# OpenNLPLab/ACR_WSSS

Hardware: NVIDIA B200
Metric: train_imgs_per_sec (higher is better)
Workload: dtype bf16

## Files before the change

acr_wsss_b200/csrc/attn_bwd_tc.cu:

```cuda
#include "attn_tc.cuh"

using namespace acr_attn;

namespace {

constexpr int NST = 3;

struct BwdSmem {
  uint8_t k[TILE_BYTES];
  uint8_t v[TILE_BYTES];
  uint8_t q[NST][TILE_BYTES];
  uint8_t d_o[NST][TILE_BYTES];
  uint8_t p[2][TILE_BYTES];
  uint8_t ds[2][TILE_BYTES];
  uint8_t dq[2][TILE_BYTES];
  float stat[2][2][BM];
  uint64_t kv_full, kv_empty, dkv_free, qdo_full[NST], qdo_empty[NST], stat_full[2], sdp_full, sdp_free, pds_full, pds_free, dq_full, dq_free;
  uint32_t tmem_base;
};
static_assert(sizeof(BwdSmem) <= 232448, "BwdSmem exceeds the 227 KB dynamic shared memory limit");

constexpr int BWD_THREADS = 512;

#ifdef ACR_BWD_TRACE
__device__ unsigned long long g_bwd_trace[4][16][8];
#define BWD_TRACE(role, tile, ev)                                                                         \
  do {                                                                                                    \
    if (blockIdx.x == 5 && (tile) < 16 && (threadIdx.x & 31) == 0) g_bwd_trace[role][tile][ev] = clock64(); \
  } while (0)
#else
#define BWD_TRACE(role, tile, ev) do { } while (0)
#endif
constexpr int REG_CTRL = 48, REG_DRAIN = 64, REG_SOFTMAX = 200;

__device__ __forceinline__ uint64_t f2_pack(float lo, float hi) {
  uint64_t r;
  asm("mov.b64 %0, {%1, %2};" : "=l"(r) : "f"(lo), "f"(hi));
  return r;
}
__device__ __forceinline__ void f2_unpack(uint64_t v, float& lo, float& hi) { asm("mov.b64 {%0, %1}, %2;" : "=f"(lo), "=f"(hi) : "l"(v)); }
__device__ __forceinline__ uint64_t f2_fma(uint64_t a, uint64_t b, uint64_t c) {
  uint64_t r;
  asm("fma.rn.f32x2 %0, %1, %2, %3;" : "=l"(r) : "l"(a), "l"(b), "l"(c));
  return r;
}
__device__ __forceinline__ uint64_t f2_mul(uint64_t a, uint64_t b) {
  uint64_t r;
  asm("mul.rn.f32x2 %0, %1, %2;" : "=l"(r) : "l"(a), "l"(b));
  return r;
}
__device__ __forceinline__ uint64_t f2_add(uint64_t a, uint64_t b) {
  uint64_t r;
  asm("add.rn.f32x2 %0, %1, %2;" : "=l"(r) : "l"(a), "l"(b));
  return r;
}
__device__ __forceinline__ void sts128(uint32_t addr, uint32_t a, uint32_t b, uint32_t c, uint32_t d) {
  asm volatile("st.shared.v4.b32 [%0], {%1, %2, %3, %4};" ::"r"(addr), "r"(a), "r"(b), "r"(c), "r"(d) : "memory");
}
template <int GMODE, bool TAIL>
__device__ __forceinline__ void bwd_softmax_tile(BwdSmem& s, uint32_t tS, uint32_t tDP, uint32_t tDS, uint32_t lane_off, int half, int row, int colbase, int N,
                                                 const float* __restrict__ grow, const uint32_t (&cwt)[16], float gw, float scale_log2, float lse2,
                                                 float dlt, float* __restrict__ rd_row0, uint32_t p_row, uint32_t ds_row, int pds_par) {
  const int nlive = TAIL ? (N - colbase) : 64;
  const uint64_t sc2 = f2_pack(scale_log2, scale_log2), nl2 = f2_pack(-lse2, -lse2), nd2 = f2_pack(-dlt, -dlt), gw2 = f2_pack(gw, gw);
  uint32_t pk[32], dk[32];
#pragma unroll
  for (int c = 0; c < 2; ++c) {
    uint32_t rs[32], rd[32];
    const bool live = !TAIL || c * 32 < nlive;
    if (live) {
      tc::tmem_ld32(tS + lane_off + half * 64 + c * 32, rs);
      tc::tmem_ld32(tDP + lane_off + half * 64 + c * 32, rd);
      tc::tmem_ld_wait();
    }
    if (c == 1) {
      tc::tc_fence_before();
      tc::mbar_arrive(&s.sdp_free);
      if (half == 0 && row < 32) BWD_TRACE(1, 15, 2);
    }
    if (!live) {
#pragma unroll
      for (int e = 0; e < 16; ++e) pk[c * 16 + e] = dk[c * 16 + e] = 0u;
    } else {
    const uint32_t* cw = cwt + c * 8;
    float g[GMODE == 1 || GMODE == 2 ? 32 : 1];
    if (GMODE == 2) {
#pragma unroll
      for (int e = 0; e < 8; ++e) {
        const float4 t = __ldg(reinterpret_cast<const float4*>(grow + c * 32) + e);
        g[4 * e] = t.x; g[4 * e + 1] = t.y; g[4 * e + 2] = t.z; g[4 * e + 3] = t.w;
      }
    } else if (GMODE == 1) {
#pragma unroll
      for (int e = 0; e < 32; ++e) g[e] = (colbase + c * 32 + e < N) ? __ldg(grow + c * 32 + e) : 0.f;
    }
    if (rd_row0 != nullptr) {
#pragma unroll
      for (int e = 0; e < 32; ++e) {
        float gv = 0.f;
        if (GMODE == 3) gv = __uint_as_float((((cw[e >> 2] >> ((e & 3) * 8)) & 0xffu) << 24));
        else if (GMODE != 0) gv = g[e];
        if (colbase + c * 32 + e < N) rd_row0[c * 32 + e] = fmaf(gv, gw, __uint_as_float(rd[e]));
      }
    }
#pragma unroll
    for (int e = 0; e < 16; ++e) {
      const int i0 = c * 32 + 2 * e;
      const uint64_t x = f2_fma(f2_pack(__uint_as_float(rs[2 * e]), __uint_as_float(rs[2 * e + 1])), sc2, nl2);
      float x0, x1;
      f2_unpack(x, x0, x1);
      float p0 = tc::fast_exp2(x0), p1 = tc::fast_exp2(x1);
      if (TAIL) {
        if (i0 >= nlive) p0 = 0.f;
        if (i0 + 1 >= nlive) p1 = 0.f;
      }
      uint64_t dp = f2_pack(__uint_as_float(rd[2 * e]), __uint_as_float(rd[2 * e + 1]));
      if (GMODE == 3) {
        float g0 = ACR_CODE_F(cw[e >> 1], (2 * e) & 3), g1 = ACR_CODE_F(cw[e >> 1], (2 * e + 1) & 3);
        if (TAIL) {
          if (i0 >= nlive) g0 = 0.f;
          if (i0 + 1 >= nlive) g1 = 0.f;
        }
        dp = f2_fma(f2_pack(g0, g1), gw2, dp);
      } else if (GMODE != 0) {
        dp = f2_fma(f2_pack(g[2 * e], g[2 * e + 1]), gw2, dp);
      }
      const uint64_t dsv = f2_mul(f2_pack(p0, p1), f2_add(dp, nd2));
      float d0, d1;
      f2_unpack(dsv, d0, d1);
      pk[c * 16 + e] = tc::pack_bf16(p0, p1);
      dk[c * 16 + e] = tc::pack_bf16(d0, d1);
    }
    }
  }
  if (pds_par >= 0) {
    if (half == 0 && row < 32) BWD_TRACE(1, 15, 3);
    tc::mbar_wait(&s.pds_free, (uint32_t)pds_par);
    tc::mbar_wait(&s.dq_full, (uint32_t)pds_par);
    tc::tc_fence_after();
    if (half == 0 && row < 32) BWD_TRACE(1, 15, 5);
  }
#pragma unroll
  for (int cc = 0; cc < 8; ++cc) {
    sts128(p_row ^ (uint32_t)(cc << 4), pk[cc * 4 + 0], pk[cc * 4 + 1], pk[cc * 4 + 2], pk[cc * 4 + 3]);
    sts128(ds_row ^ (uint32_t)(cc << 4), dk[cc * 4 + 0], dk[cc * 4 + 1], dk[cc * 4 + 2], dk[cc * 4 + 3]);
  }
  tc::tmem_st16(tDS + lane_off + half * 32, dk);
  tc::tmem_st16(tDS + lane_off + half * 32 + 16, dk + 16);
  tc::tmem_st_wait();
}

struct SoftmaxArgs {
  uint32_t tS, tDP, tDS, lane_off;
  int half, row, colbase, N, H, ntiles, b, h;
  const float* g_mean;
  long long g_bs, g_ld;
  float* g_row0;
  const unsigned char* code;
  long long code_bs, code_ld;
  float w_cls2, w_aff2, invH, scale_log2;
  uint32_t p_row, ds_row, swz;
};

template <int GMODE, bool TAIL>
__device__ __forceinline__ void bwd_softmax_loop(BwdSmem& s, const SoftmaxArgs& a, int T0) {
  const int row = a.row, N = a.N;
  const int wq = row & ~31;
  uint32_t cwn[16];
  auto load_codes = [&](int i) {
    const uint4* src = reinterpret_cast<const uint4*>(a.code + (size_t)a.b * a.code_bs + (size_t)min(i * BM + row, N - 1) * a.code_ld + a.colbase);
#pragma unroll
    for (int v = 0; v < 4; ++v) {
      uint4 t = make_uint4(0u, 0u, 0u, 0u);
      if (!TAIL || a.colbase + v * 16 < N) t = __ldg(src + v);
      cwn[v * 4 + 0] = t.x; cwn[v * 4 + 1] = t.y; cwn[v * 4 + 2] = t.z; cwn[v * 4 + 3] = t.w;
    }
  };
  if (GMODE == 3) load_codes(0);
  for (int i = 0; i < a.ntiles; ++i) {
    uint32_t cw[16];
    if (GMODE == 3) {
#pragma unroll
      for (int v = 0; v < 16; ++v) cw[v] = cwn[v];
      if (i + 1 < a.ntiles) load_codes(i + 1);
    }
    const int q0 = i * BM;
    const int T = T0 + i;
    const int pds_par = (T > 0) ? ((T - 1) & 1) : -1;
    const int qi = q0 + row;
    const bool rows_live = q0 + wq < N;
    float lse2 = INFINITY, dlt = 0.f;
    if (rows_live) {
      tc::mbar_wait(&s.stat_full[T & 1], (T >> 1) & 1);
      lse2 = s.stat[T & 1][0][row];
      dlt = s.stat[T & 1][1][row];
    }
    if (a.half == 0 && row < 32) BWD_TRACE(1, i, 0);
    tc::mbar_wait(&s.sdp_full, T & 1);
    tc::tc_fence_after();
    if (a.half == 0 && row < 32) BWD_TRACE(1, i, 1);
    if (!rows_live) {
      tc::tc_fence_before();
      tc::mbar_arrive(&s.sdp_free);
      if (pds_par >= 0) {
        tc::mbar_wait(&s.pds_free, (uint32_t)pds_par);
        tc::mbar_wait(&s.dq_full, (uint32_t)pds_par);
        tc::tc_fence_after();
      }
#pragma unroll
      for (int cc = 0; cc < 8; ++cc) {
        sts128(a.p_row ^ (uint32_t)(cc << 4), 0u, 0u, 0u, 0u);
        sts128(a.ds_row ^ (uint32_t)(cc << 4), 0u, 0u, 0u, 0u);
      }
      {
        uint32_t z[16];
#pragma unroll
        for (int e = 0; e < 16; ++e) z[e] = 0u;
        tc::tmem_st16(a.tDS + a.lane_off + a.half * 32, z);
        tc::tmem_st16(a.tDS + a.lane_off + a.half * 32 + 16, z);
        tc::tmem_st_wait();
      }
    } else {
      const float* grow = (GMODE == 1 || GMODE == 2) ? a.g_mean + (size_t)a.b * a.g_bs + (size_t)min(qi, N - 1) * a.g_ld + a.colbase : nullptr;
      float* rd_row0 = (a.g_row0 != nullptr && qi == 0) ? a.g_row0 + ((size_t)a.b * a.H + a.h) * N + a.colbase : nullptr;
      const float gw = (GMODE == 3) ? ((qi == 0) ? a.w_cls2 : a.w_aff2) : a.invH;
      bwd_softmax_tile<GMODE, TAIL>(s, a.tS, a.tDP, a.tDS, a.lane_off, a.half, row, a.colbase, N, grow, cw, gw, a.scale_log2, lse2, dlt, rd_row0,
                                    a.p_row, a.ds_row, pds_par);
    }
    tc::fence_proxy_async_smem();
    tc::mbar_arrive(&s.pds_full);
    if (a.half == 0 && row < 32) BWD_TRACE(1, i, 4);
  }
}

struct Items {
  int kt_full, nfull, nthin;
  __device__ bool at(int c, int G, int k, int& kvt, int& hb, bool& tail) const {
    const int nf = nfull > c ? (nfull - c + G - 1) / G : 0;
    if (k < nf) {
      const int f = c + k * G;
      kvt = f % kt_full;
      hb = f / kt_full;
      tail = false;
      return true;
    }
    k -= nf;
    const int cr = G - 1 - c;
    const int nt = nthin > cr ? (nthin - cr + G - 1) / G : 0;
    if (k < nt) {
      kvt = kt_full;
      hb = cr + k * G;
      tail = true;
      return true;
    }
    return false;
  }
};

__global__ void __launch_bounds__(BWD_THREADS, 1)
attn_bwd_kernel(const __grid_constant__ CUtensorMap tmap_qkv, const __grid_constant__ CUtensorMap tmap_do,
                const __grid_constant__ CUtensorMap tmap_dq,
                const float* __restrict__ lse, const float* __restrict__ delta, const float* __restrict__ g_mean, long long g_bs,
                long long g_ld, GCode gc, __nv_bfloat16* __restrict__ d_qkv, float* __restrict__ g_row0, int* __restrict__ dq_bad, float dq_lim,
                int N, int H, int HB, float scale, float scale_log2) {
  extern __shared__ __align__(1024) uint8_t smem_raw[];
  BwdSmem& s = *reinterpret_cast<BwdSmem*>(smem_raw);
  const int warp = threadIdx.x >> 5, lane = threadIdx.x & 31;
  const int ntiles = (N + BM - 1) / BM;
  const bool has_code = gc.ptr != nullptr;
  const int G = gridDim.x, cta = blockIdx.x;
  Items items;
  items.kt_full = N / BN;
  items.nfull = items.kt_full * HB;
  items.nthin = (N % BN) ? HB : 0;

  if (warp == 0 && lane == 0) {
    if (tc::smem_u32(smem_raw) & 1023u) __trap();
    tc::prefetch_tmap(&tmap_qkv);
    tc::prefetch_tmap(&tmap_do);
    tc::prefetch_tmap(&tmap_dq);
    tc::mbar_init(&s.kv_full, 1);
    tc::mbar_init(&s.kv_empty, 1);
    tc::mbar_init(&s.dkv_free, 128);
    for (int i = 0; i < NST; ++i) {
      tc::mbar_init(&s.qdo_full[i], 1);
      tc::mbar_init(&s.qdo_empty[i], 1);
    }
    for (int i = 0; i < 2; ++i) tc::mbar_init(&s.stat_full[i], 64);
    tc::mbar_init(&s.sdp_full, 1);
    tc::mbar_init(&s.sdp_free, 256);
    tc::mbar_init(&s.pds_full, 256);
    tc::mbar_init(&s.pds_free, 1);
    tc::mbar_init(&s.dq_full, 1);
    tc::mbar_init(&s.dq_free, 128);
    tc::fence_barrier_init();
  }
  if (warp == 2) tc::tmem_alloc<512>(&s.tmem_base);
  tc::tc_fence_before();
  __syncthreads();
  tc::tc_fence_after();
  if (warp == 0) BWD_TRACE(3, 0, 0);
  const uint32_t tmem = s.tmem_base;
  const uint32_t tS = tmem, tDP = tmem + 128, tDV = tmem + 256, tDK = tmem + 320, tDQ = tmem + 384, tDS = tmem + 448;

  if (warp < 4) {
    tc::reg_dealloc<REG_CTRL>();
    if (warp == 0) {
      int T = 0, kvt, hb;
      bool tail;
      for (int k = 0; items.at(cta, G, k, kvt, hb, tail); ++k) {
        const int h = hb % H, b = hb / H, kv0 = kvt * BN;
        tc::mbar_wait(&s.kv_empty, (k & 1) ^ 1);
        if (tc::elect_one()) {
          tc::mbar_arrive_expect_tx(&s.kv_full, 2 * TILE_BYTES);
          tc::tma_load_4d(s.k, &tmap_qkv, &s.kv_full, 0, H + h, kv0, b);
          tc::tma_load_4d(s.v, &tmap_qkv, &s.kv_full, 0, 2 * H + h, kv0, b);
        }
        __syncwarp();
        for (int i = 0; i < ntiles; ++i, ++T) {
          const int st = T % NST;
          tc::mbar_wait(&s.qdo_empty[st], ((T / NST) & 1) ^ 1);
          if (tc::elect_one()) {
            tc::mbar_arrive_expect_tx(&s.qdo_full[st], 2 * TILE_BYTES);
            tc::tma_load_4d(s.q[st], &tmap_qkv, &s.qdo_full[st], 0, h, i * BM, b);
            tc::tma_load_4d(s.d_o[st], &tmap_do, &s.qdo_full[st], 0, h, i * BM, b);
          }
          __syncwarp();
        }
      }
    } else if (warp == 1) {
      const uint64_t kd_k = tc::smem_desc_sw128(tc::smem_u32(s.k), 16, 1024);
      const uint64_t vd_k = tc::smem_desc_sw128(tc::smem_u32(s.v), 16, 1024);
      const uint64_t kd_mn = tc::smem_desc_sw128(tc::smem_u32(s.k), 1024, 1024);
      const uint64_t pd_mn = tc::smem_desc_sw128(tc::smem_u32(s.p[0]), TILE_BYTES, 1024);
      const uint64_t dsd_mn = tc::smem_desc_sw128(tc::smem_u32(s.ds[0]), TILE_BYTES, 1024);
      auto issue_scores = [&](int T) {
        const int st = T % NST;
        tc::mbar_wait(&s.qdo_full[st], (T / NST) & 1);
        tc::tc_fence_after();
        BWD_TRACE(0, T, 0);
        const uint64_t qd = tc::smem_desc_sw128(tc::smem_u32(s.q[st]), 16, 1024), dod = tc::smem_desc_sw128(tc::smem_u32(s.d_o[st]), 16, 1024);
        if (tc::elect_one()) {
#pragma unroll
          for (int ks = 0; ks < HD / 16; ++ks) tc::mma_ss_off(tS, qd, ks * 2, kd_k, ks * 2, IDESC_S, ks > 0);
#pragma unroll
          for (int ks = 0; ks < HD / 16; ++ks) tc::mma_ss_off(tDP, dod, ks * 2, vd_k, ks * 2, IDESC_S, ks > 0);
          tc::tc_commit(&s.sdp_full);
        }
        __syncwarp();
      };
      int T = 0, kvt, hb;
      bool tail;
      for (int k = 0; items.at(cta, G, k, kvt, hb, tail); ++k) {
        tc::mbar_wait(&s.kv_full, k & 1);
        if (T > 0) tc::mbar_wait(&s.sdp_free, (T - 1) & 1);
        issue_scores(T);
        for (int i = 0; i < ntiles; ++i, ++T) {
          const int st = T % NST;
          if (i + 1 < ntiles) {
            tc::mbar_wait(&s.sdp_free, T & 1);
            issue_scores(T + 1);
          }
          const uint64_t qd_mn = tc::smem_desc_sw128(tc::smem_u32(s.q[st]), 1024, 1024), dod_mn = tc::smem_desc_sw128(tc::smem_u32(s.d_o[st]), 1024, 1024);
          BWD_TRACE(0, T, 1);
          tc::mbar_wait(&s.pds_full, T & 1);
          BWD_TRACE(0, T, 2);
          if (T >= 1) tc::mbar_wait(&s.dq_free, (T - 1) & 1);
          if (i == 0 && k > 0) tc::mbar_wait(&s.dkv_free, (k - 1) & 1);
          tc::tc_fence_after();
          const uint32_t acc = (i > 0) ? 1u : 0u;
          if (tc::elect_one()) {
#pragma unroll
            for (int ks = 0; ks < BM / 16; ++ks)
              tc::mma_ss_off(tDK, dsd_mn, ks * 128, qd_mn, ks * 128, IDESC_DQ, acc | (ks > 0));
#pragma unroll
            for (int ks = 0; ks < BM / 16; ++ks)
              tc::mma_ss_off(tDV, pd_mn, ks * 128, dod_mn, ks * 128, IDESC_DQ, acc | (ks > 0));
            tc::tc_commit(&s.pds_free);
            tc::tc_commit(&s.qdo_empty[st]);
#pragma unroll
            for (int ks = 0; ks < BN / 16; ++ks)
              tc::mma_ts_off(tDQ, tDS + ks * 8, kd_mn, ks * 128, IDESC_PV, ks > 0);
            tc::tc_commit(&s.dq_full);
            if (i + 1 == ntiles) tc::tc_commit(&s.kv_empty);
          }
          __syncwarp();
          BWD_TRACE(0, T, 3);
        }
      }
    } else {
      const int which = warp - 2;
      int T = 0, kvt, hb;
      bool tail;
      for (int k = 0; items.at(cta, G, k, kvt, hb, tail); ++k) {
        const float* src = (which == 0 ? lse : delta) + (size_t)hb * N;
        for (int i = 0; i < ntiles; ++i, ++T) {
          if (T >= 2) tc::mbar_wait(&s.qdo_empty[(T - 2) % NST], ((T - 2) / NST) & 1);
          float v[4];
#pragma unroll
          for (int q = 0; q < 4; ++q) {
            const int qi = i * BM + q * 32 + lane;
            v[q] = (qi < N) ? __ldg(src + qi) : (which == 0 ? INFINITY : 0.f);
          }
#pragma unroll
          for (int q = 0; q < 4; ++q) s.stat[T & 1][which][q * 32 + lane] = (which == 0) ? v[q] * kLog2e : v[q];
          tc::mbar_arrive(&s.stat_full[T & 1]);
        }
      }
    }
  } else if (warp < 12) {
    tc::reg_alloc<REG_SOFTMAX>();
    const int we = warp - 4;
    const int row = (warp & 3) * 32 + lane;
    const int half = we >> 2;
    const uint32_t lane_off = (uint32_t)((warp & 3) * 32) << 16;
    const float invH = 1.f / (float)H;
    const bool g_vec = (g_mean != nullptr) && ((g_ld & 3) == 0) && ((g_bs & 3) == 0) && ((reinterpret_cast<uintptr_t>(g_mean) & 15) == 0);
    float w_cls2 = 0.f, w_aff2 = 0.f;
    if (has_code) {
      const float sc = gc.scale ? __ldg(gc.scale) : 1.f;
      w_cls2 = 2.f * invH * sc * gc.w_cls;
      w_aff2 = 2.f * invH * sc * gc.w_aff;
    }
    const uint32_t swz = (uint32_t)(row & 7) << 4;
    const uint32_t p_row = (tc::smem_u32(s.p[half]) + row * 128) ^ swz, ds_row = (tc::smem_u32(s.ds[half]) + row * 128) ^ swz;
    int T = 0, k = 0, kvt, hb;
    bool tail;
    auto run = [&](auto body, bool want_tail) {
      while (items.at(cta, G, k, kvt, hb, tail) && tail == want_tail) {
        const SoftmaxArgs sa{tS, tDP, tDS, lane_off, half, row, kvt * BN + half * 64, N, H, ntiles, hb / H, hb % H, g_mean, g_bs, g_ld, g_row0,
                             gc.ptr, gc.bs, gc.ld, w_cls2, w_aff2, invH, scale_log2, p_row, ds_row, swz};
        body(sa, T);
        T += ntiles;
        ++k;
      }
    };
    if (has_code) {
      run([&](const SoftmaxArgs& sa, int T0) { bwd_softmax_loop<3, false>(s, sa, T0); }, false);
      run([&](const SoftmaxArgs& sa, int T0) { bwd_softmax_loop<3, true>(s, sa, T0); }, true);
    } else if (g_mean != nullptr && g_vec) {
      run([&](const SoftmaxArgs& sa, int T0) { bwd_softmax_loop<2, false>(s, sa, T0); }, false);
      run([&](const SoftmaxArgs& sa, int T0) { bwd_softmax_loop<1, true>(s, sa, T0); }, true);
    } else if (g_mean != nullptr) {
      run([&](const SoftmaxArgs& sa, int T0) { bwd_softmax_loop<1, true>(s, sa, T0); }, false);
      run([&](const SoftmaxArgs& sa, int T0) { bwd_softmax_loop<1, true>(s, sa, T0); }, true);
    } else {
      run([&](const SoftmaxArgs& sa, int T0) { bwd_softmax_loop<0, false>(s, sa, T0); }, false);
      run([&](const SoftmaxArgs& sa, int T0) { bwd_softmax_loop<0, true>(s, sa, T0); }, true);
    }
  } else {
    tc::reg_dealloc<REG_DRAIN>();
    const int row = (warp & 3) * 32 + lane;
    const uint32_t lane_off = (uint32_t)((warp & 3) * 32) << 16;
    const bool leader = (warp == 12 && lane == 0);
    const uint32_t dq_row = (tc::smem_u32(s.dq[0]) + row * 128) ^ ((uint32_t)(row & 7) << 4);
    uint32_t r[32];
    auto drain_box = [&](int base, int buf, int col, int i, int hb) {
      if (leader) asm volatile("cp.async.bulk.wait_group.read 1;" ::: "memory");
      asm volatile("bar.sync 3, 128;" ::: "memory");
      bool bad = false;
#pragma unroll
      for (int e = 0; e < 8; ++e) {
        const float fa = __uint_as_float(r[base + 2 * e]) * kDqFix, fb = __uint_as_float(r[base + 2 * e + 1]) * kDqFix;
        const bool oka = fabsf(fa) < dq_lim, okb = fabsf(fb) < dq_lim;
        bad |= !(oka && okb);
        const long long a = oka ? __float2ll_rn(fa) : 0ll, b = okb ? __float2ll_rn(fb) : 0ll;
        sts128((dq_row + buf * TILE_BYTES) ^ (uint32_t)(e << 4), (uint32_t)a, (uint32_t)((unsigned long long)a >> 32), (uint32_t)b,
               (uint32_t)((unsigned long long)b >> 32));
      }
      if (bad && i * BM + row < N) dq_bad[(size_t)hb * N + i * BM + row] = 1;
      tc::fence_proxy_async_smem();
      asm volatile("bar.sync 3, 128;" ::: "memory");
      if (leader) {
        asm volatile("cp.reduce.async.bulk.tensor.3d.global.shared::cta.add.tile.bulk_group [%0, {%2, %3, %4}], [%1];" ::"l"(
                         reinterpret_cast<uint64_t>(&tmap_dq)),
                     "r"(tc::smem_u32(s.dq[buf])), "r"(col), "r"(i * BM), "r"(hb)
                     : "memory");
        asm volatile("cp.async.bulk.commit_group;" ::: "memory");
      }
    };
    int T = 0, kvt, hb;
    bool tail;
    for (int k = 0; items.at(cta, G, k, kvt, hb, tail); ++k) {
      for (int i = 0; i < ntiles; ++i, ++T) {
        if (warp == 12) BWD_TRACE(2, T, 0);
        tc::mbar_wait(&s.dq_full, T & 1);
        tc::tc_fence_after();
        if (warp == 12) BWD_TRACE(2, T, 1);
        tc::tmem_ld32(tDQ + lane_off, r);
        tc::tmem_ld_wait();
        drain_box(0, 0, 0, i, hb);
        drain_box(16, 1, 16, i, hb);
        tc::tmem_ld32(tDQ + lane_off + 32, r);
        tc::tmem_ld_wait();
        tc::tc_fence_before();
        tc::mbar_arrive(&s.dq_free);
        if (warp == 12) BWD_TRACE(2, T, 2);
        drain_box(0, 0, 32, i, hb);
        drain_box(16, 1, 48, i, hb);
        if (leader) BWD_TRACE(2, T, 3);
      }
      const int h = hb % H, b = hb / H, kv0 = kvt * BN;
      const bool kv_ok = (kv0 + row) < N;
      const size_t E = (size_t)H * HD;
      __nv_bfloat16* base = d_qkv + ((size_t)b * N + min(kv0 + row, N - 1)) * 3 * E + (size_t)h * HD;
#pragma unroll
      for (int part = 0; part < 4; ++part) {
        const bool is_k = part >= 2;
        tc::tmem_ld32((is_k ? tDK : tDV) + lane_off + (part & 1) * 32, r);
        tc::tmem_ld_wait();
        if (kv_ok) {
          const float sc = is_k ? scale : 1.f;
          __nv_bfloat16* dst = base + (is_k ? 1 : 2) * E + (part & 1) * 32;
#pragma unroll
          for (int c = 0; c < 4; ++c) {
            uint4 v;
            v.x = tc::pack_bf16(__uint_as_float(r[c * 8 + 0]) * sc, __uint_as_float(r[c * 8 + 1]) * sc);
            v.y = tc::pack_bf16(__uint_as_float(r[c * 8 + 2]) * sc, __uint_as_float(r[c * 8 + 3]) * sc);
            v.z = tc::pack_bf16(__uint_as_float(r[c * 8 + 4]) * sc, __uint_as_float(r[c * 8 + 5]) * sc);
            v.w = tc::pack_bf16(__uint_as_float(r[c * 8 + 6]) * sc, __uint_as_float(r[c * 8 + 7]) * sc);
            reinterpret_cast<uint4*>(dst)[c] = v;
          }
        }
      }
      tc::tc_fence_before();
      tc::mbar_arrive(&s.dkv_free);
    }
    if (leader) asm volatile("cp.async.bulk.wait_group 0;" ::: "memory");
  }
  tc::tc_fence_before();
  __syncthreads();
  if (warp == 0) BWD_TRACE(3, 0, 1);
  if (warp == 2) {
    tc::tc_fence_after();
    tc::tmem_dealloc<512>(tmem);
  }
}

}

namespace acr_attn {

int launch_attn_bwd(const CUtensorMap& tmap_qkv, const CUtensorMap& tmap_do, const CUtensorMap& tmap_dq, const float* lse, const float* delta,
                    const float* g_mean, long long g_bs, long long g_ld, const GCode& gc, __nv_bfloat16* d_qkv, float* g_row0,
                    int* dq_bad, int B, int N, int H, float scale, cudaStream_t st) {
  const size_t smem = sizeof(BwdSmem);
  static bool attr_set[64] = {false};
  if (int e = set_max_smem(attn_bwd_kernel, smem, attr_set)) return e;
  static int sms[64] = {0};
  int dev = 0;
  ACR_CUDA(cudaGetDevice(&dev));
  if (dev < 0 || dev >= 64) dev = 0;
  if (!sms[dev]) ACR_CUDA(cudaDeviceGetAttribute(&sms[dev], cudaDevAttrMultiProcessorCount, dev));
  const int kt = (N + BN - 1) / BN;
  const long long nitems = (long long)kt * H * B;
  const unsigned grid = (unsigned)(nitems < sms[dev] ? nitems : sms[dev]);
  acr::KernelTimer kt_("attn_bwd_kernel", st);
  attn_bwd_kernel<<<grid, BWD_THREADS, smem, st>>>(tmap_qkv, tmap_do, tmap_dq, lse, delta, g_mean, g_bs, g_ld, gc, d_qkv, g_row0, dq_bad,
                                                    dq_fix_limit(kt), N, H, H * B, scale, scale * kLog2e);
  return acr::check_launch("attn_bwd_kernel");
}

}

#ifdef ACR_BWD_TRACE
extern "C" void acr_bwd_trace_read(unsigned long long* host ) { cudaMemcpyFromSymbol(host, g_bwd_trace, sizeof(g_bwd_trace)); }
#endif
```

acr_wsss_b200/csrc/attn_tc.cu:

```cuda
#include "attn_tc.cuh"
#include <cstdlib>

using namespace acr_attn;

namespace {

struct FwdSmem {
  uint8_t q[TILE_BYTES];
  uint8_t k[2][TILE_BYTES];
  uint8_t v[2][TILE_BYTES];
  float mx[2][2][BM];
  float lsum[2][BM];
  uint64_t q_full, kv_full[2], kv_empty[2], s_full, s_free, p_full, o_full;
  uint32_t tmem_base;
};

constexpr float kRescaleThreshold = 8.f;
constexpr int FWD_THREADS = 384;
__device__ __forceinline__ void fwd_pair_sync(int quad) {
  switch (quad) {
    case 0: asm volatile("bar.sync 1, 64;" ::: "memory"); break;
    case 1: asm volatile("bar.sync 2, 64;" ::: "memory"); break;
    case 2: asm volatile("bar.sync 3, 64;" ::: "memory"); break;
    default: asm volatile("bar.sync 4, 64;" ::: "memory"); break;
  }
}
__global__ void __launch_bounds__(FWD_THREADS, 2)
attn_fwd_kernel(const __grid_constant__ CUtensorMap tmap_qkv, __nv_bfloat16* __restrict__ out, float* __restrict__ lse,
                int N, int H, float scale_log2) {
  extern __shared__ uint8_t smem_raw[];
  FwdSmem& s = *reinterpret_cast<FwdSmem*>((reinterpret_cast<uintptr_t>(smem_raw) + 1023) & ~(uintptr_t)1023);
  const int warp = threadIdx.x >> 5, lane = threadIdx.x & 31;
  const int q0 = blockIdx.x * BM, h = blockIdx.y, b = blockIdx.z;
  const int ntiles = (N + BN - 1) / BN;

  if (warp == 0 && lane == 0) {
    tc::prefetch_tmap(&tmap_qkv);
    tc::mbar_init(&s.q_full, 1);
    for (int i = 0; i < 2; ++i) { tc::mbar_init(&s.kv_full[i], 1); tc::mbar_init(&s.kv_empty[i], 1); }
    tc::mbar_init(&s.s_full, 1);
    tc::mbar_init(&s.s_free, 256);
    tc::mbar_init(&s.p_full, 256);
    tc::mbar_init(&s.o_full, 1);
    tc::fence_barrier_init();
  }
  if (warp == 2) tc::tmem_alloc<256>(&s.tmem_base);
  tc::tc_fence_before();
  __syncthreads();
  tc::tc_fence_after();
  const uint32_t tmem = s.tmem_base;
  const uint32_t tS = tmem, tP = tmem + 128, tO = tmem + 192;

  if (warp == 0) {
    tc::reg_dealloc<40>();
    if (tc::elect_one()) {
      tc::mbar_arrive_expect_tx(&s.q_full, TILE_BYTES);
      tc::tma_load_4d(s.q, &tmap_qkv, &s.q_full, 0, h, q0, b);
    }
    __syncwarp();
    for (int j = 0; j < ntiles; ++j) {
      const int st = j & 1;
      tc::mbar_wait(&s.kv_empty[st], ((j >> 1) & 1) ^ 1);
      if (tc::elect_one()) {
        tc::mbar_arrive_expect_tx(&s.kv_full[st], 2 * TILE_BYTES);
        tc::tma_load_4d(s.k[st], &tmap_qkv, &s.kv_full[st], 0, H + h, j * BN, b);
        tc::tma_load_4d(s.v[st], &tmap_qkv, &s.kv_full[st], 0, 2 * H + h, j * BN, b);
      }
      __syncwarp();
    }
  } else if (warp == 1) {
    tc::reg_dealloc<40>();
    tc::mbar_wait(&s.q_full, 0);
    const uint64_t qd = tc::smem_desc_sw128(tc::smem_u32(s.q), 16, 1024);
    auto issue_s = [&](int j) {
      const uint64_t kd = tc::smem_desc_sw128(tc::smem_u32(s.k[j & 1]), 16, 1024);
      if (tc::elect_one()) {
#pragma unroll
        for (int ks = 0; ks < HD / 16; ++ks) tc::mma_ss_off(tS, qd, ks * 2, kd, ks * 2, IDESC_S, ks > 0);
        tc::tc_commit(&s.s_full);
      }
      __syncwarp();
    };
    tc::mbar_wait(&s.kv_full[0], 0);
    tc::tc_fence_after();
    issue_s(0);
    for (int j = 0; j < ntiles; ++j) {
      const int st = j & 1;
      if (j + 1 < ntiles) {
        tc::mbar_wait(&s.kv_full[(j + 1) & 1], ((j + 1) >> 1) & 1);
        tc::mbar_wait(&s.s_free, j & 1);
        tc::tc_fence_after();
        issue_s(j + 1);
      }
      tc::mbar_wait(&s.p_full, j & 1);
      tc::tc_fence_after();
      const uint64_t vd = tc::smem_desc_sw128(tc::smem_u32(s.v[st]), 1024, 1024);
      if (tc::elect_one()) {
#pragma unroll
        for (int ks = 0; ks < BN / 16; ++ks) tc::mma_ts_off(tO, tP + ks * 8, vd, ks * 128, IDESC_PV, (j > 0) || (ks > 0));
        tc::tc_commit(&s.o_full);
        tc::tc_commit(&s.kv_empty[st]);
      }
      __syncwarp();
    }
  } else if (warp < 4) {
    tc::reg_dealloc<40>();
  } else {
    tc::reg_alloc<96>();
    const int half = (warp - 4) >> 2;
    const int quad = warp & 3;
    const int row = quad * 32 + lane;
    const uint32_t lane_off = (uint32_t)(quad * 32) << 16;
    const int cb = half * 64;
    float m = -INFINITY, l = 0.f;
    uint32_t r[32];
    const bool rows_live = q0 + quad * 32 < N;
    for (int j = 0; j < ntiles; ++j) {
      tc::mbar_wait(&s.s_full, j & 1);
      tc::tc_fence_after();
      if (!rows_live) {
        tc::tc_fence_before();
        tc::mbar_arrive(&s.s_free);
        tc::mbar_arrive(&s.p_full);
        tc::mbar_wait(&s.p_full, j & 1);
        continue;
      }
      const int ncols = min(BN, N - j * BN);
      const bool full = (ncols == BN);
      float mx = -INFINITY;
#pragma unroll
      for (int c = 0; c < 2; ++c) {
        const int c0 = cb + c * 32;
        if (c0 < ncols) {
          tc::tmem_ld32(tS + lane_off + c0, r);
          tc::tmem_ld_wait();
          if (full) {
#pragma unroll
            for (int i = 0; i < 32; ++i) mx = fmaxf(mx, __uint_as_float(r[i]));
          } else {
#pragma unroll
            for (int i = 0; i < 32; ++i) mx = fmaxf(mx, (c0 + i < ncols) ? __uint_as_float(r[i]) : -INFINITY);
          }
        }
      }
      s.mx[j & 1][half][row] = mx;
      fwd_pair_sync(quad);
      mx = fmaxf(mx, s.mx[j & 1][half ^ 1][row]);
      if (j > 0) {
        tc::mbar_wait(&s.o_full, (j - 1) & 1);
        tc::tc_fence_after();
      }
      if (j == 0) {
        m = mx;
      } else {
        const bool need = (mx - m) * scale_log2 > kRescaleThreshold;
        if (__any_sync(0xffffffffu, need)) {
          const float alpha = need ? tc::fast_exp2((m - mx) * scale_log2) : 1.f;
          if (need) { m = mx; l *= alpha; }
          tc::tmem_ld32(tO + lane_off + half * 32, r);
          tc::tmem_ld_wait();
#pragma unroll
          for (int i = 0; i < 32; ++i) r[i] = __float_as_uint(__uint_as_float(r[i]) * alpha);
          tc::tmem_st16(tO + lane_off + half * 32, r);
          tc::tmem_st16(tO + lane_off + half * 32 + 16, r + 16);
        }
      }
      const float ms = m * scale_log2;
      const uint64_t sc2 = tc::f2_pack(scale_log2, scale_log2), nms2 = tc::f2_pack(-ms, -ms);
      uint64_t rs2 = tc::f2_pack(0.f, 0.f);
#pragma unroll
      for (int c = 0; c < 2; ++c) {
        const int c0 = cb + c * 32;
        const bool any = c0 < ncols;
        if (any) {
          tc::tmem_ld32(tS + lane_off + c0, r);
          tc::tmem_ld_wait();
        }
        if (c == 1) {
          tc::tc_fence_before();
          tc::mbar_arrive(&s.s_free);
        }
        uint32_t pk[16];
        if (any) {
#pragma unroll
          for (int i = 0; i < 16; ++i) {
            float x0, x1;
            tc::f2_unpack(tc::f2_fma(tc::f2_pack(__uint_as_float(r[2 * i]), __uint_as_float(r[2 * i + 1])), sc2, nms2), x0, x1);
            float p0 = tc::fast_exp2(x0), p1 = tc::fast_exp2(x1);
            if (!full) {
              if (c0 + 2 * i >= ncols) p0 = 0.f;
              if (c0 + 2 * i + 1 >= ncols) p1 = 0.f;
            }
            rs2 = tc::f2_add(rs2, tc::f2_pack(p0, p1));
            pk[i] = tc::pack_bf16(p0, p1);
          }
        } else {
#pragma unroll
          for (int i = 0; i < 16; ++i) pk[i] = 0u;
        }
        tc::tmem_st16(tP + lane_off + half * 32 + c * 16, pk);
      }
      tc::tmem_st_wait();
      tc::tc_fence_before();
      tc::mbar_arrive(&s.p_full);
      float rs_lo, rs_hi;
      tc::f2_unpack(rs2, rs_lo, rs_hi);
      l += rs_lo + rs_hi;
    }
    if (rows_live) {
      s.lsum[half][row] = l;
      fwd_pair_sync(quad);
      l += s.lsum[half ^ 1][row];
      tc::mbar_wait(&s.o_full, (ntiles - 1) & 1);
      tc::tc_fence_after();
      tc::tmem_ld32(tO + lane_off + half * 32, r);
      tc::tmem_ld_wait();
      if (q0 + row < N) {
        const float inv = 1.f / l;
        __nv_bfloat16* dst = out + ((size_t)b * N + q0 + row) * ((size_t)H * HD) + (size_t)h * HD + half * 32;
#pragma unroll
        for (int c = 0; c < 4; ++c) {
          uint4 v;
          v.x = tc::pack_bf16(__uint_as_float(r[c * 8 + 0]) * inv, __uint_as_float(r[c * 8 + 1]) * inv);
          v.y = tc::pack_bf16(__uint_as_float(r[c * 8 + 2]) * inv, __uint_as_float(r[c * 8 + 3]) * inv);
          v.z = tc::pack_bf16(__uint_as_float(r[c * 8 + 4]) * inv, __uint_as_float(r[c * 8 + 5]) * inv);
          v.w = tc::pack_bf16(__uint_as_float(r[c * 8 + 6]) * inv, __uint_as_float(r[c * 8 + 7]) * inv);
          reinterpret_cast<uint4*>(dst)[c] = v;
        }
        if (half == 0) lse[((size_t)b * H + h) * N + q0 + row] = (m * scale_log2 + log2f(l)) * kLn2;
      }
    }
  }
  tc::tc_fence_before();
  __syncthreads();
  if (warp == 2) {
    tc::tc_fence_after();
    tc::tmem_dealloc<256>(tmem);
  }
}

constexpr int MEAN_STAGES = 3;
constexpr int MEAN_SW_SLICES = 4;
struct MeanSmem {
  uint8_t qk[MEAN_STAGES][2][TILE_BYTES];
  float lse2[MEAN_MAX_H][BM];
  float part[MEAN_SW_SLICES][MEAN_MAX_H][BM];
  uint64_t full[MEAN_STAGES], empty[MEAN_STAGES], t_full[2], t_empty[2];
  uint32_t tmem_base;
};
constexpr int STAGE_LD = 129;
static_assert(sizeof(float) * BM * STAGE_LD <= sizeof(uint8_t) * MEAN_STAGES * 2 * TILE_BYTES, "staging tile must fit");

constexpr int MEAN_SW = 16;
static_assert(MEAN_SW == 4 * MEAN_SW_SLICES, "slices of the softmax warps");
constexpr int MEAN_COLS = BN / (MEAN_SW / 4);
constexpr int MEAN_THREADS = 128 + MEAN_SW * 32;

template <int MODE>
__global__ void __launch_bounds__(MEAN_THREADS, 1)
attn_mean_kernel(const __grid_constant__ CUtensorMap tmap_qkv, const float* __restrict__ lse, float* __restrict__ mean,
                 long long mean_bs, long long mean_ld, GCode gc, float* __restrict__ p_row0, int N, int H, float scale_log2) {
  extern __shared__ uint8_t smem_raw[];
  MeanSmem& s = *reinterpret_cast<MeanSmem*>((reinterpret_cast<uintptr_t>(smem_raw) + 1023) & ~(uintptr_t)1023);
  const int warp = threadIdx.x >> 5, lane = threadIdx.x & 31;
  const int kv0 = blockIdx.x * BN, q0 = blockIdx.y * BM, b = blockIdx.z;

  if (warp == 0 && lane == 0) {
    tc::prefetch_tmap(&tmap_qkv);
    for (int i = 0; i < MEAN_STAGES; ++i) { tc::mbar_init(&s.full[i], 1); tc::mbar_init(&s.empty[i], 1); }
    for (int i = 0; i < 2; ++i) { tc::mbar_init(&s.t_full[i], 1); tc::mbar_init(&s.t_empty[i], MEAN_SW * 32); }
    tc::fence_barrier_init();
  }
  if (warp == 2) tc::tmem_alloc<256>(&s.tmem_base);
  tc::tc_fence_before();
  __syncthreads();
  tc::tc_fence_after();
  const uint32_t tmem = s.tmem_base;

  if (warp == 0) {
    for (int h = 0; h < H; ++h) {
      const int st = h % MEAN_STAGES;
      tc::mbar_wait(&s.empty[st], ((h / MEAN_STAGES) & 1) ^ 1);
      if (tc::elect_one()) {
        tc::mbar_arrive_expect_tx(&s.full[st], 2 * TILE_BYTES);
        tc::tma_load_4d(s.qk[st][0], &tmap_qkv, &s.full[st], 0, h, q0, b);
        tc::tma_load_4d(s.qk[st][1], &tmap_qkv, &s.full[st], 0, H + h, kv0, b);
      }
      __syncwarp();
    }
  } else if (warp == 1) {
    for (int h = 0; h < H; ++h) {
      const int st = h % MEAN_STAGES, ab = h & 1;
      tc::mbar_wait(&s.full[st], (h / MEAN_STAGES) & 1);
      tc::mbar_wait(&s.t_empty[ab], ((h >> 1) & 1) ^ 1);
      tc::tc_fence_after();
      const uint64_t qd = tc::smem_desc_sw128(tc::smem_u32(s.qk[st][0]), 16, 1024), kd = tc::smem_desc_sw128(tc::smem_u32(s.qk[st][1]), 16, 1024);
      if (tc::elect_one()) {
#pragma unroll
        for (int ks = 0; ks < HD / 16; ++ks) tc::mma_ss_off(tmem + ab * 128, qd, ks * 2, kd, ks * 2, IDESC_S, ks > 0);
        tc::tc_commit(&s.empty[st]);
        tc::tc_commit(&s.t_full[ab]);
      }
      __syncwarp();
    }
  } else if (warp >= 4) {
    const int we = warp - 4;
    const int row = (warp & 3) * 32 + lane;
    const int slice = we >> 2;
    const int sidx = we * 32 + lane;
    const uint32_t lane_off = (uint32_t)((warp & 3) * 32) << 16;
    const bool row_ok = (q0 + row) < N;
    const int col0 = kv0 + slice * MEAN_COLS;
    float acc[MEAN_COLS];
    const float invH = 1.f / (float)H;
    if (MODE == 0) {
#pragma unroll
      for (int i = 0; i < MEAN_COLS; ++i) acc[i] = 0.f;
    } else if (gc.ptr == nullptr) {
      const float* grow = mean + (size_t)b * mean_bs + (size_t)(q0 + row) * mean_ld + col0;
#pragma unroll
      for (int i = 0; i < MEAN_COLS; ++i) acc[i] = (row_ok && col0 + i < N) ? __ldg(grow + i) * invH : 0.f;
    } else {
      const float w2 = gcode_weight(gc, q0 + row, invH);
      const uint4* crow = reinterpret_cast<const uint4*>(gc.ptr + (size_t)b * gc.bs + (size_t)min(q0 + row, N - 1) * gc.ld + col0);
#pragma unroll
      for (int v = 0; v < MEAN_COLS / 16; ++v) {
        const uint4 t = __ldg(crow + v);
        const uint32_t w[4] = {t.x, t.y, t.z, t.w};
#pragma unroll
        for (int j = 0; j < 4; ++j)
#pragma unroll
          for (int k = 0; k < 4; ++k) {
            const int i = v * 16 + j * 4 + k;
            acc[i] = (row_ok && col0 + i < N) ? ACR_CODE_F(w[j], k) * w2 : 0.f;
          }
      }
    }
    {
      constexpr int HSTEP = MEAN_SW * 32 / BM;
      const int rr = sidx & (BM - 1);
      const bool ok = (q0 + rr) < N;
      const float* lp = lse + (size_t)b * H * N + q0 + rr;
      for (int h0 = sidx / BM; h0 < H; h0 += HSTEP * 4) {
        float v[4];
#pragma unroll
        for (int k = 0; k < 4; ++k) v[k] = (ok && h0 + HSTEP * k < H) ? __ldg(lp + (size_t)(h0 + HSTEP * k) * N) : INFINITY;
#pragma unroll
        for (int k = 0; k < 4; ++k)
          if (h0 + HSTEP * k < H) s.lse2[h0 + HSTEP * k][rr] = v[k] * kLog2e;
      }
    }
    asm volatile("bar.sync 1, %0;" ::"n"(MEAN_SW * 32) : "memory");
    const bool tail = (kv0 + BN > N);
    const bool row0_warp = (MODE == 0) && (p_row0 != nullptr) && (q0 == 0) && ((warp & 3) == 0);
    const bool live = (q0 + (warp & 3) * 32 < N) && (col0 < N);
    uint32_t r[32];
    for (int h = 0; h < H; ++h) {
      const int ab = h & 1;
      const float lse2 = s.lse2[h][row];
      tc::mbar_wait(&s.t_full[ab], (h >> 1) & 1);
      tc::tc_fence_after();
      float part = 0.f;
#pragma unroll
      for (int c = 0; c < MEAN_COLS / 32; ++c) {
        const int colbase = col0 + c * 32;
        if (!live || (tail && colbase >= N)) break;
        tc::tmem_ld32(tmem + ab * 128 + lane_off + slice * MEAN_COLS + c * 32, r);
        tc::tmem_ld_wait();
        if (!tail) {
          const uint64_t sc2 = tc::f2_pack(scale_log2, scale_log2), nl2 = tc::f2_pack(-lse2, -lse2);
          uint64_t part2 = tc::f2_pack(0.f, 0.f);
#pragma unroll
          for (int i = 0; i < 32; i += 2) {
            float x0, x1;
            tc::f2_unpack(tc::f2_fma(tc::f2_pack(__uint_as_float(r[i]), __uint_as_float(r[i + 1])), sc2, nl2), x0, x1);
            const float p0 = tc::fast_exp2(x0), p1 = tc::fast_exp2(x1);
            const uint64_t pp = tc::f2_pack(p0, p1), aa = tc::f2_pack(acc[c * 32 + i], acc[c * 32 + i + 1]);
            if (MODE == 0) {
              tc::f2_unpack(tc::f2_add(aa, pp), acc[c * 32 + i], acc[c * 32 + i + 1]);
              r[i] = __float_as_uint(p0); r[i + 1] = __float_as_uint(p1);
            } else {
              part2 = tc::f2_fma(pp, aa, part2);
            }
          }
          if (MODE == 1) { float a0, a1; tc::f2_unpack(part2, a0, a1); part += a0 + a1; }
        } else {
#pragma unroll
          for (int i = 0; i < 32; ++i) {
            float p = tc::fast_exp2(fmaf(__uint_as_float(r[i]), scale_log2, -lse2));
            if (colbase + i >= N) p = 0.f;
            if (MODE == 0) { acc[c * 32 + i] += p; r[i] = __float_as_uint(p); } else part = fmaf(p, acc[c * 32 + i], part);
          }
        }
        if (row0_warp && lane == 0) {
          float* dst0 = p_row0 + ((size_t)b * H + h) * N + colbase;
#pragma unroll
          for (int i = 0; i < 32; ++i)
            if (colbase + i < N) dst0[i] = __uint_as_float(r[i]);
        }
      }
      tc::tc_fence_before();
      tc::mbar_arrive(&s.t_empty[ab]);
      if (MODE == 1) s.part[slice][h][row] = part;
    }
    if (MODE == 1) {
      asm volatile("bar.sync 1, %0;" ::"n"(MEAN_SW * 32) : "memory");
      float* plane = p_row0 + (size_t)blockIdx.x * gridDim.z * H * N;
      for (int idx = sidx; idx < H * BM; idx += MEAN_SW * 32) {
        const int hh = idx / BM, rr = idx % BM;
        if (q0 + rr < N) {
          float v = 0.f;
#pragma unroll
          for (int sl = 0; sl < MEAN_SW_SLICES; ++sl) v += s.part[sl][hh][rr];
          plane[((size_t)b * H + hh) * N + q0 + rr] = v;
        }
      }
    }
    if (MODE == 0) {
    float* stage = reinterpret_cast<float*>(&s.qk[0][0][0]);
#pragma unroll
    for (int i = 0; i < MEAN_COLS; ++i) stage[row * STAGE_LD + slice * MEAN_COLS + i] = acc[i] * invH;
    asm volatile("bar.sync 1, %0;" ::"n"(MEAN_SW * 32) : "memory");
    float* dst = mean + (size_t)b * mean_bs;
    constexpr int RPW = BM / MEAN_SW;
#pragma unroll 1
    for (int r4 = we * RPW; r4 < we * RPW + RPW; r4 += 4) {
      if (q0 + r4 >= N) break;
      float v[4][4];
#pragma unroll
      for (int u = 0; u < 4; ++u)
#pragma unroll
        for (int cc = 0; cc < 4; ++cc) v[u][cc] = stage[(r4 + u) * STAGE_LD + cc * 32 + lane];
#pragma unroll
      for (int u = 0; u < 4; ++u) {
        if (q0 + r4 + u < N) {
#pragma unroll
          for (int cc = 0; cc < 4; ++cc) {
            const int col = cc * 32 + lane;
            if (kv0 + col < N) dst[(size_t)(q0 + r4 + u) * N + kv0 + col] = v[u][cc];
          }
        }
      }
    }
    }
  }
  tc::tc_fence_before();
  __syncthreads();
  if (warp == 2) {
    tc::tc_fence_after();
    tc::tmem_dealloc<256>(tmem);
  }
}

}

namespace acr_attn {
EncodeTiledFn get_encode_fn() {
  static EncodeTiledFn fn = nullptr;
  if (!fn) {
    void* p = nullptr;
    cudaDriverEntryPointQueryResult qres;
    if (cudaGetDriverEntryPoint("cuTensorMapEncodeTiled", &p, cudaEnableDefault, &qres) != cudaSuccess || qres != cudaDriverEntryPointSuccess)
      return nullptr;
    fn = (EncodeTiledFn)p;
  }
  return fn;
}

int make_tmap(CUtensorMap* m, const void* base, int B, int N, int SH, int D) {
  EncodeTiledFn fn = get_encode_fn();
  ACR_REQUIRE(fn != nullptr, ACR_E_NOSM100, "cuTensorMapEncodeTiled unavailable");
  cuuint64_t dims[4] = {(cuuint64_t)D, (cuuint64_t)SH, (cuuint64_t)N, (cuuint64_t)B};
  cuuint64_t strides[3] = {(cuuint64_t)D * 2, (cuuint64_t)SH * D * 2, (cuuint64_t)N * SH * D * 2};
  cuuint32_t box[4] = {(cuuint32_t)D, 1, (cuuint32_t)BM, 1};
  cuuint32_t estr[4] = {1, 1, 1, 1};
  CUresult r = fn(m, CU_TENSOR_MAP_DATA_TYPE_BFLOAT16, 4, const_cast<void*>(base), dims, strides, box, estr, CU_TENSOR_MAP_INTERLEAVE_NONE,
                  CU_TENSOR_MAP_SWIZZLE_128B, CU_TENSOR_MAP_L2_PROMOTION_L2_256B, CU_TENSOR_MAP_FLOAT_OOB_FILL_NONE);
  ACR_REQUIRE(r == CUDA_SUCCESS, ACR_E_INVAL, "cuTensorMapEncodeTiled failed (%d)", (int)r);
  return 0;
}

}

extern "C" int acr_attn_fwd_bf16(const void* qkv, int B, int N, int H, int D, float scale,
                                 void* out, float* lse, float* attn_mean, long long mean_batch_stride,
                                 float* p_row0, void* stream) {
  ACR_REQUIRE(qkv && out && lse, ACR_E_INVAL, "acr_attn_fwd_bf16: null pointer");
  ACR_REQUIRE(B > 0 && N > 0 && H > 0, ACR_E_INVAL, "acr_attn_fwd_bf16: bad shape");
  ACR_REQUIRE(D == HD, ACR_E_INVAL, "acr_attn_fwd_bf16: head dim %d unsupported (64 only)", D);
  ACR_REQUIRE(B <= 65535 && H <= MEAN_MAX_H, ACR_E_INVAL, "acr_attn_fwd_bf16: B <= 65535 and H <= %d required", MEAN_MAX_H);
  ACR_REQUIRE(((uintptr_t)qkv & 15) == 0 && ((uintptr_t)out & 15) == 0, ACR_E_ALIGN, "acr_attn_fwd_bf16: qkv/out must be 16-byte aligned");
  ACR_REQUIRE(p_row0 == nullptr || attn_mean != nullptr, ACR_E_INVAL, "acr_attn_fwd_bf16: p_row0 needs attn_mean");
  ACR_REQUIRE(acr_device_is_sm100(), ACR_E_NOSM100, "acr_attn_fwd_bf16: needs an sm_100 device");
  cudaStream_t st = (cudaStream_t)stream;
  CUtensorMap tmap;
  if (int e = make_tmap(&tmap, qkv, B, N, 3 * H, D)) return e;
  const float scale_log2 = scale * kLog2e;
  const int qt = (N + BM - 1) / BM, kt = (N + BN - 1) / BN;
  {
    const size_t smem = sizeof(FwdSmem) + 1024;
    static bool attr_set[64] = {false};
    if (int e = set_max_smem(attn_fwd_kernel, smem, attr_set)) return e;
    dim3 grid(qt, H, B);
    acr::KernelTimer kt_("attn_fwd_kernel", st);
    attn_fwd_kernel<<<grid, FWD_THREADS, smem, st>>>(tmap, (__nv_bfloat16*)out, lse, N, H, scale_log2);
    if (int e = acr::check_launch("attn_fwd_kernel")) return e;
  }
  if (attn_mean) {
    const size_t smem = sizeof(MeanSmem) + 1024;
    static bool attr_set[64] = {false};
    if (int e = set_max_smem(attn_mean_kernel<0>, smem, attr_set)) return e;
    dim3 grid(kt, qt, B);
    acr::KernelTimer kt_("attn_mean_kernel", st);
    attn_mean_kernel<0><<<grid, MEAN_THREADS, smem, st>>>(tmap, lse, attn_mean, mean_batch_stride, (long long)N, GCode{}, p_row0, N, H, scale_log2);
    if (int e = acr::check_launch("attn_mean_kernel")) return e;
  }
  return 0;
}


namespace {


__global__ void __launch_bounds__(256)
bwd_delta_kernel(const __nv_bfloat16* __restrict__ out, const __nv_bfloat16* __restrict__ d_out, const float* __restrict__ part,
                 int nparts, float* __restrict__ delta, float4* __restrict__ dq_acc, int* __restrict__ dq_bad, long long rows, int N, int H) {
  const int lane = threadIdx.x & 31;
  const long long t = ((long long)blockIdx.x * (blockDim.x >> 5) + (threadIdx.x >> 5)) * 4 + (lane >> 3);
  const bool ok = t < rows;
  float acc = 0.f;
  if (ok) {
    const uint4 a = __ldg(reinterpret_cast<const uint4*>(out + t * HD) + (lane & 7));
    const uint4 d = __ldg(reinterpret_cast<const uint4*>(d_out + t * HD) + (lane & 7));
    const __nv_bfloat162* a2 = reinterpret_cast<const __nv_bfloat162*>(&a);
    const __nv_bfloat162* d2 = reinterpret_cast<const __nv_bfloat162*>(&d);
#pragma unroll
    for (int i = 0; i < 4; ++i) {
      const float2 fa = __bfloat1622float2(a2[i]), fd = __bfloat1622float2(d2[i]);
      acc = fmaf(fa.x, fd.x, acc);
      acc = fmaf(fa.y, fd.y, acc);
    }
    const float4 z = make_float4(0.f, 0.f, 0.f, 0.f);
#pragma unroll
    for (int m = 0; m < 4; ++m) dq_acc[t * (HD / 2) + m * 8 + (lane & 7)] = z;
  }
  acc += __shfl_xor_sync(0xffffffffu, acc, 1);
  acc += __shfl_xor_sync(0xffffffffu, acc, 2);
  acc += __shfl_xor_sync(0xffffffffu, acc, 4);
  if (ok && (lane & 7) == 0) {
    const int h = (int)(t % H);
    const long long bn = t / H;
    const int n = (int)(bn % N), b = (int)(bn / N);
    const size_t idx = ((size_t)b * H + h) * N + n;
    for (int k = 0; k < nparts; ++k) acc += __ldg(part + (size_t)k * rows + idx);
    delta[idx] = acc;
    dq_bad[idx] = 0;
  }
}

__global__ void __launch_bounds__(256)
bwd_dq_convert_kernel(const long long* __restrict__ dq_acc, const int* __restrict__ dq_bad, __nv_bfloat16* __restrict__ d_qkv, int B, int N,
                      int H, float scale) {
  const long long t = (long long)blockIdx.x * blockDim.x + threadIdx.x;
  if (t >= (long long)B * H * N * (HD / 8)) return;
  const int c = (int)(t % (HD / 8));
  const long long row = t / (HD / 8);
  const int n = (int)(row % N);
  const int h = (int)((row / N) % H);
  const int b = (int)(row / ((long long)N * H));
  const longlong2* src = reinterpret_cast<const longlong2*>(dq_acc + row * HD + c * 8);
  const float sc = __ldg(dq_bad + row) ? __int_as_float(0x7fc00000) : scale * kDqUnfix;
  float x[8];
#pragma unroll
  for (int j = 0; j < 4; ++j) {
    const longlong2 q = __ldg(src + j);
    x[2 * j] = __ll2float_rn(q.x) * sc;
    x[2 * j + 1] = __ll2float_rn(q.y) * sc;
  }
  uint4 v;
  v.x = tc::pack_bf16(x[0], x[1]);
  v.y = tc::pack_bf16(x[2], x[3]);
  v.z = tc::pack_bf16(x[4], x[5]);
  v.w = tc::pack_bf16(x[6], x[7]);
  *reinterpret_cast<uint4*>(d_qkv + (((size_t)b * N + n) * 3 + 0) * ((size_t)H * HD) + (size_t)h * HD + c * 8) = v;
}

}

extern "C" size_t acr_attn_bwd_bf16_workspace(int B, int N, int H, int D) {
  if (B <= 0 || N <= 0 || H <= 0 || D <= 0) return 0;
  const size_t rows = (size_t)B * H * N, kt = (N + BN - 1) / BN;
  return acr::align_up(rows * sizeof(float), 256) + acr::align_up(rows * D * sizeof(long long), 256) + acr::align_up(kt * rows * sizeof(float), 256) +
         acr::align_up(rows * sizeof(int), 256);
}

extern "C" int acr_attn_bwd_bf16(const void* qkv, const void* out, const float* lse, const void* d_out,
                                 int B, int N, int H, int D, float scale,
                                 const float* g_mean, long long g_batch_stride, long long g_row_stride,
                                 const unsigned char* g_code, long long code_batch_stride, long long code_row_stride,
                                 float w_cls, float w_aff, const float* g_scale,
                                 void* d_qkv, float* g_row0, void* workspace, size_t workspace_bytes, void* stream) {
  ACR_REQUIRE(qkv && out && lse && d_out && d_qkv && workspace, ACR_E_INVAL, "acr_attn_bwd_bf16: null pointer");
  ACR_REQUIRE(B > 0 && N > 0 && H > 0, ACR_E_INVAL, "acr_attn_bwd_bf16: bad shape");
  ACR_REQUIRE(D == HD, ACR_E_INVAL, "acr_attn_bwd_bf16: head dim %d unsupported (64 only)", D);
  ACR_REQUIRE(B <= 65535 && H <= MEAN_MAX_H, ACR_E_INVAL, "acr_attn_bwd_bf16: B <= 65535 and H <= %d required", MEAN_MAX_H);
  ACR_REQUIRE(g_mean == nullptr || g_row_stride >= N, ACR_E_INVAL, "acr_attn_bwd_bf16: g_row_stride < N");
  ACR_REQUIRE(g_mean == nullptr || g_code == nullptr, ACR_E_INVAL, "acr_attn_bwd_bf16: give g_mean OR g_code");
  ACR_REQUIRE(g_code == nullptr || ((code_row_stride % 128) == 0 && code_row_stride >= (long long)((N + 127) / 128) * 128 &&
                                    (code_batch_stride % 16) == 0 && ((uintptr_t)g_code & 15) == 0),
              ACR_E_ALIGN, "acr_attn_bwd_bf16: g_code rows must be 128-byte padded and 16-byte aligned");
  const GCode gc{g_code, code_batch_stride, code_row_stride, w_cls, w_aff, g_scale};
  ACR_REQUIRE(((uintptr_t)qkv & 15) == 0 && ((uintptr_t)out & 15) == 0 && ((uintptr_t)d_out & 15) == 0 && ((uintptr_t)d_qkv & 15) == 0,
              ACR_E_ALIGN, "acr_attn_bwd_bf16: tensors must be 16-byte aligned");
  ACR_REQUIRE(((uintptr_t)workspace & 255) == 0, ACR_E_ALIGN, "acr_attn_bwd_bf16: workspace must be 256-byte aligned");
  ACR_REQUIRE(workspace_bytes >= acr_attn_bwd_bf16_workspace(B, N, H, D), ACR_E_NOMEM, "acr_attn_bwd_bf16: workspace too small");
  ACR_REQUIRE(acr_device_is_sm100(), ACR_E_NOSM100, "acr_attn_bwd_bf16: needs an sm_100 device");
  cudaStream_t st = (cudaStream_t)stream;
  const size_t rows = (size_t)B * H * N;
  const int qt = (N + BM - 1) / BM, kt = (N + BN - 1) / BN;
  float* delta = (float*)workspace;
  long long* dq_acc = (long long*)((char*)workspace + acr::align_up(rows * sizeof(float), 256));
  float* delta_part = (float*)((char*)dq_acc + acr::align_up(rows * D * sizeof(long long), 256));
  int* dq_bad = (int*)((char*)delta_part + acr::align_up((size_t)kt * rows * sizeof(float), 256));
  CUtensorMap tmap_qkv, tmap_do, tmap_dq;
  if (int e = make_tmap(&tmap_qkv, qkv, B, N, 3 * H, D)) return e;
  if (int e = make_tmap(&tmap_do, d_out, B, N, H, D)) return e;
  {
    EncodeTiledFn fn = get_encode_fn();
    ACR_REQUIRE(fn != nullptr, ACR_E_NOSM100, "cuTensorMapEncodeTiled unavailable");
    cuuint64_t dims[3] = {(cuuint64_t)HD, (cuuint64_t)N, (cuuint64_t)B * H};
    cuuint64_t strides[2] = {(cuuint64_t)HD * 8, (cuuint64_t)N * HD * 8};
    cuuint32_t box[3] = {16, (cuuint32_t)BM, 1};
    cuuint32_t estr[3] = {1, 1, 1};
    CUresult r = fn(&tmap_dq, CU_TENSOR_MAP_DATA_TYPE_UINT64, 3, dq_acc, dims, strides, box, estr, CU_TENSOR_MAP_INTERLEAVE_NONE,
                    CU_TENSOR_MAP_SWIZZLE_128B, CU_TENSOR_MAP_L2_PROMOTION_NONE, CU_TENSOR_MAP_FLOAT_OOB_FILL_NONE);
    ACR_REQUIRE(r == CUDA_SUCCESS, ACR_E_INVAL, "cuTensorMapEncodeTiled(dq) failed (%d)", (int)r);
  }
  const float scale_log2 = scale * kLog2e;

  const bool with_g = g_mean || g_code;
  if (with_g) {
    const size_t smem = sizeof(MeanSmem) + 1024;
    static bool attr_set[64] = {false};
    if (int e = set_max_smem(attn_mean_kernel<1>, smem, attr_set)) return e;
    dim3 grid(kt, qt, B);
    acr::KernelTimer kt_("attn_delta_kernel", st);
    attn_mean_kernel<1><<<grid, MEAN_THREADS, smem, st>>>(tmap_qkv, lse, const_cast<float*>(g_mean), g_batch_stride, g_row_stride, gc, delta_part, N, H, scale_log2);
    if (int e = acr::check_launch("attn_mean_kernel<1>")) return e;
  }
  bwd_delta_kernel<<<(unsigned)((rows + 31) / 32), 256, 0, st>>>((const __nv_bfloat16*)out, (const __nv_bfloat16*)d_out, delta_part,
                                                               with_g ? kt : 0, delta, reinterpret_cast<float4*>(dq_acc), dq_bad, (long long)rows, N, H);
  if (int e = acr::check_launch("bwd_delta_kernel")) return e;
  if (int e = launch_attn_bwd(tmap_qkv, tmap_do, tmap_dq, lse, delta, g_mean, g_batch_stride, g_row_stride, gc, (__nv_bfloat16*)d_qkv, g_row0, dq_bad, B, N, H, scale, st))
    return e;
  const long long nconv = (long long)rows * (HD / 8);
  bwd_dq_convert_kernel<<<(unsigned)((nconv + 255) / 256), 256, 0, st>>>(dq_acc, dq_bad, (__nv_bfloat16*)d_qkv, B, N, H, scale);
  return acr::check_launch("bwd_dq_convert_kernel");
}
```

Before: 585.6.

## Restructure attention backward to transposed S/dP with P kept in TMEM

```diff
diff --git a/acr_wsss_b200/csrc/attn_bwd_tc.cu b/acr_wsss_b200/csrc/attn_bwd_tc.cu
--- a/acr_wsss_b200/csrc/attn_bwd_tc.cu
+++ b/acr_wsss_b200/csrc/attn_bwd_tc.cu
@@ -11,11 +11,11 @@
   uint8_t v[TILE_BYTES];
   uint8_t q[NST][TILE_BYTES];
   uint8_t d_o[NST][TILE_BYTES];
-  uint8_t p[2][TILE_BYTES];
-  uint8_t ds[2][TILE_BYTES];
+  uint8_t ds[2][2][TILE_BYTES];
   uint8_t dq[2][TILE_BYTES];
   float stat[2][2][BM];
-  uint64_t kv_full, kv_empty, dkv_free, qdo_full[NST], qdo_empty[NST], stat_full[2], sdp_full, sdp_free, pds_full, pds_free, dq_full, dq_free;
+  uint64_t kv_full, kv_empty, dkv_free, qdo_full[NST], qdo_empty[NST], stat_full[2], s_full, dp_full, p_full, ds_full, p_done, dk_done,
+      ds_free[2], dq_full[2], dq_free[2];
   uint32_t tmem_base;
 };
 static_assert(sizeof(BwdSmem) <= 232448, "BwdSmem exceeds the 227 KB dynamic shared memory limit");
@@ -33,146 +33,147 @@
 #endif
 constexpr int REG_CTRL = 48, REG_DRAIN = 64, REG_SOFTMAX = 200;
 
-__device__ __forceinline__ uint64_t f2_pack(float lo, float hi) {
-  uint64_t r;
-  asm("mov.b64 %0, {%1, %2};" : "=l"(r) : "f"(lo), "f"(hi));
-  return r;
-}
-__device__ __forceinline__ void f2_unpack(uint64_t v, float& lo, float& hi) { asm("mov.b64 {%0, %1}, %2;" : "=f"(lo), "=f"(hi) : "l"(v)); }
-__device__ __forceinline__ uint64_t f2_fma(uint64_t a, uint64_t b, uint64_t c) {
-  uint64_t r;
-  asm("fma.rn.f32x2 %0, %1, %2, %3;" : "=l"(r) : "l"(a), "l"(b), "l"(c));
-  return r;
-}
+using tc::f2_pack;
+using tc::f2_unpack;
+using tc::f2_fma;
+using tc::f2_add;
 __device__ __forceinline__ uint64_t f2_mul(uint64_t a, uint64_t b) {
   uint64_t r;
   asm("mul.rn.f32x2 %0, %1, %2;" : "=l"(r) : "l"(a), "l"(b));
   return r;
 }
-__device__ __forceinline__ uint64_t f2_add(uint64_t a, uint64_t b) {
-  uint64_t r;
-  asm("add.rn.f32x2 %0, %1, %2;" : "=l"(r) : "l"(a), "l"(b));
-  return r;
-}
 __device__ __forceinline__ void sts128(uint32_t addr, uint32_t a, uint32_t b, uint32_t c, uint32_t d) {
   asm volatile("st.shared.v4.b32 [%0], {%1, %2, %3, %4};" ::"r"(addr), "r"(a), "r"(b), "r"(c), "r"(d) : "memory");
 }
-template <int GMODE, bool TAIL>
-__device__ __forceinline__ void bwd_softmax_tile(BwdSmem& s, uint32_t tS, uint32_t tDP, uint32_t tDS, uint32_t lane_off, int half, int row, int colbase, int N,
-                                                 const float* __restrict__ grow, const uint32_t (&cwt)[16], float gw, float scale_log2, float lse2,
-                                                 float dlt, float* __restrict__ rd_row0, uint32_t p_row, uint32_t ds_row, int pds_par) {
-  const int nlive = TAIL ? (N - colbase) : 64;
-  const uint64_t sc2 = f2_pack(scale_log2, scale_log2), nl2 = f2_pack(-lse2, -lse2), nd2 = f2_pack(-dlt, -dlt), gw2 = f2_pack(gw, gw);
-  uint32_t pk[32], dk[32];
-#pragma unroll
-  for (int c = 0; c < 2; ++c) {
-    uint32_t rs[32], rd[32];
-    const bool live = !TAIL || c * 32 < nlive;
-    if (live) {
-      tc::tmem_ld32(tS + lane_off + half * 64 + c * 32, rs);
-      tc::tmem_ld32(tDP + lane_off + half * 64 + c * 32, rd);
-      tc::tmem_ld_wait();
-    }
-    if (c == 1) {
-      tc::tc_fence_before();
-      tc::mbar_arrive(&s.sdp_free);
-      if (half == 0 && row < 32) BWD_TRACE(1, 15, 2);
-    }
-    if (!live) {
-#pragma unroll
-      for (int e = 0; e < 16; ++e) pk[c * 16 + e] = dk[c * 16 + e] = 0u;
-    } else {
-    const uint32_t* cw = cwt + c * 8;
-    float g[GMODE == 1 || GMODE == 2 ? 32 : 1];
-    if (GMODE == 2) {
-#pragma unroll
-      for (int e = 0; e < 8; ++e) {
-        const float4 t = __ldg(reinterpret_cast<const float4*>(grow + c * 32) + e);
-        g[4 * e] = t.x; g[4 * e + 1] = t.y; g[4 * e + 2] = t.z; g[4 * e + 3] = t.w;
-      }
-    } else if (GMODE == 1) {
-#pragma unroll
-      for (int e = 0; e < 32; ++e) g[e] = (colbase + c * 32 + e < N) ? __ldg(grow + c * 32 + e) : 0.f;
-    }
-    if (rd_row0 != nullptr) {
-#pragma unroll
-      for (int e = 0; e < 32; ++e) {
-        float gv = 0.f;
-        if (GMODE == 3) gv = __uint_as_float((((cw[e >> 2] >> ((e & 3) * 8)) & 0xffu) << 24));
-        else if (GMODE != 0) gv = g[e];
-        if (colbase + c * 32 + e < N) rd_row0[c * 32 + e] = fmaf(gv, gw, __uint_as_float(rd[e]));
-      }
-    }
-#pragma unroll
-    for (int e = 0; e < 16; ++e) {
-      const int i0 = c * 32 + 2 * e;
-      const uint64_t x = f2_fma(f2_pack(__uint_as_float(rs[2 * e]), __uint_as_float(rs[2 * e + 1])), sc2, nl2);
-      float x0, x1;
-      f2_unpack(x, x0, x1);
-      float p0 = tc::fast_exp2(x0), p1 = tc::fast_exp2(x1);
-      if (TAIL) {
-        if (i0 >= nlive) p0 = 0.f;
-        if (i0 + 1 >= nlive) p1 = 0.f;
-      }
-      uint64_t dp = f2_pack(__uint_as_float(rd[2 * e]), __uint_as_float(rd[2 * e + 1]));
-      if (GMODE == 3) {
-        float g0 = ACR_CODE_F(cw[e >> 1], (2 * e) & 3), g1 = ACR_CODE_F(cw[e >> 1], (2 * e + 1) & 3);
-        if (TAIL) {
-          if (i0 >= nlive) g0 = 0.f;
-          if (i0 + 1 >= nlive) g1 = 0.f;
-        }
-        dp = f2_fma(f2_pack(g0, g1), gw2, dp);
-      } else if (GMODE != 0) {
-        dp = f2_fma(f2_pack(g[2 * e], g[2 * e + 1]), gw2, dp);
-      }
-      const uint64_t dsv = f2_mul(f2_pack(p0, p1), f2_add(dp, nd2));
-      float d0, d1;
-      f2_unpack(dsv, d0, d1);
-      pk[c * 16 + e] = tc::pack_bf16(p0, p1);
-      dk[c * 16 + e] = tc::pack_bf16(d0, d1);
-    }
-    }
-  }
-  if (pds_par >= 0) {
-    if (half == 0 && row < 32) BWD_TRACE(1, 15, 3);
-    tc::mbar_wait(&s.pds_free, (uint32_t)pds_par);
-    tc::mbar_wait(&s.dq_full, (uint32_t)pds_par);
-    tc::tc_fence_after();
-    if (half == 0 && row < 32) BWD_TRACE(1, 15, 5);
-  }
-#pragma unroll
-  for (int cc = 0; cc < 8; ++cc) {
-    sts128(p_row ^ (uint32_t)(cc << 4), pk[cc * 4 + 0], pk[cc * 4 + 1], pk[cc * 4 + 2], pk[cc * 4 + 3]);
-    sts128(ds_row ^ (uint32_t)(cc << 4), dk[cc * 4 + 0], dk[cc * 4 + 1], dk[cc * 4 + 2], dk[cc * 4 + 3]);
-  }
-  tc::tmem_st16(tDS + lane_off + half * 32, dk);
-  tc::tmem_st16(tDS + lane_off + half * 32 + 16, dk + 16);
-  tc::tmem_st_wait();
-}
+__device__ __forceinline__ uint64_t lds_pair(const float* p) { return *reinterpret_cast<const uint64_t*>(p); }
 
 struct SoftmaxArgs {
-  uint32_t tS, tDP, tDS, lane_off;
-  int half, row, colbase, N, H, ntiles, b, h;
-  const float* g_mean;
-  long long g_bs, g_ld;
+  uint32_t tS, tDP, lane_off;
+  int half, row, key, N, H, ntiles, b, h;
+  bool warp_live, key_live;
+  const float* g_col;
+  long long g_ld;
   float* g_row0;
   const unsigned char* code;
-  long long code_bs, code_ld;
   float w_cls2, w_aff2, invH, scale_log2;
-  uint32_t p_row, ds_row, swz;
+  uint32_t ds_row;
 };
 
-template <int GMODE, bool TAIL>
+template <int GMODE, bool KEYTAIL>
+__device__ __forceinline__ void bwd_softmax_tile(BwdSmem& s, const SoftmaxArgs& a, int i, int T, const uint32_t (&cw)[16]) {
+  const int q0 = i * BM + a.half * 64;
+  const int nlive = a.N - q0;
+  const float* nlse = &s.stat[T & 1][0][a.half * 64];
+  const float* ndlt = &s.stat[T & 1][1][a.half * 64];
+  const uint64_t sc2 = f2_pack(a.scale_log2, a.scale_log2);
+  const float wa = (GMODE == 3) ? a.w_aff2 : a.invH;
+  const float w0 = (GMODE == 3 && q0 == 0) ? a.w_cls2 : wa;
+  const uint64_t gw2 = f2_pack(wa, wa), gw2_first = f2_pack(w0, wa);
+  float p[64];
+
+  tc::mbar_wait(&s.s_full, T & 1);
+  tc::tc_fence_after();
+  if (a.half == 0 && a.row < 32) BWD_TRACE(1, i, 0);
+  if (a.warp_live) {
+#pragma unroll
+    for (int c = 0; c < 2; ++c) {
+      uint32_t pk[16];
+      if (c * 32 < nlive) {
+        uint32_t rs[32];
+        tc::tmem_ld32(a.tS + a.lane_off + a.half * 64 + c * 32, rs);
+        tc::tmem_ld_wait();
+#pragma unroll
+        for (int e = 0; e < 16; ++e) {
+          const uint64_t x = f2_fma(f2_pack(__uint_as_float(rs[2 * e]), __uint_as_float(rs[2 * e + 1])), sc2, lds_pair(nlse + c * 32 + 2 * e));
+          float x0, x1;
+          f2_unpack(x, x0, x1);
+          p[c * 32 + 2 * e] = tc::fast_exp2(x0);
+          p[c * 32 + 2 * e + 1] = tc::fast_exp2(x1);
+          pk[e] = tc::pack_bf16(p[c * 32 + 2 * e], p[c * 32 + 2 * e + 1]);
+        }
+      } else {
+#pragma unroll
+        for (int e = 0; e < 16; ++e) pk[e] = 0u;
+#pragma unroll
+        for (int e = 0; e < 32; ++e) p[c * 32 + e] = 0.f;
+      }
+      tc::tmem_st16(a.tS + a.lane_off + a.half * 64 + c * 16, pk);
+    }
+    tc::tmem_st_wait();
+  }
+  tc::tc_fence_before();
+  tc::mbar_arrive(&s.p_full);
+  if (a.half == 0 && a.row < 32) BWD_TRACE(1, i, 1);
+
+  tc::mbar_wait(&s.dp_full, T & 1);
+  if (a.half == 0 && a.row < 32) BWD_TRACE(1, i, 2);
+  if (T >= 2) tc::mbar_wait(&s.ds_free[T & 1], ((T - 2) >> 1) & 1);
+  tc::tc_fence_after();
+  if (a.half == 0 && a.row < 32) BWD_TRACE(1, i, 3);
+  const uint32_t ds_row = a.ds_row + (uint32_t)(T & 1) * (2 * TILE_BYTES);
+  if (a.warp_live) {
+#pragma unroll
+    for (int c = 0; c < 2; ++c) {
+      uint32_t dk[16];
+      if (c * 32 < nlive) {
+        uint32_t rd[32];
+        tc::tmem_ld32(a.tDP + a.lane_off + a.half * 64 + c * 32, rd);
+        float g[GMODE == 1 ? 32 : 1];
+        if (GMODE == 1) {
+#pragma unroll
+          for (int e = 0; e < 32; ++e) g[e] = (c * 32 + e < nlive) ? __ldg(a.g_col + (size_t)(q0 + c * 32 + e) * a.g_ld) : 0.f;
+        }
+        tc::tmem_ld_wait();
+        if (c == 0 && a.g_row0 != nullptr && q0 == 0 && a.key_live) {
+          float gv = 0.f;
+          if (GMODE == 3) gv = ACR_CODE_F(cw[0], 0);
+          else if (GMODE == 1) gv = g[0];
+          a.g_row0[((size_t)a.b * a.H + a.h) * a.N + a.key] = fmaf(gv, w0, __uint_as_float(rd[0]));
+        }
+        const uint32_t* cwc = cw + c * 8;
+#pragma unroll
+        for (int e = 0; e < 16; ++e) {
+          uint64_t dp = f2_pack(__uint_as_float(rd[2 * e]), __uint_as_float(rd[2 * e + 1]));
+          const uint64_t gw = (c == 0 && e == 0) ? gw2_first : gw2;
+          if (GMODE == 3) dp = f2_fma(f2_pack(ACR_CODE_F(cwc[e >> 1], (2 * e) & 3), ACR_CODE_F(cwc[e >> 1], (2 * e + 1) & 3)), gw, dp);
+          else if (GMODE == 1) dp = f2_fma(f2_pack(g[2 * e], g[2 * e + 1]), gw, dp);
+          const uint64_t dsv = f2_mul(f2_pack(p[c * 32 + 2 * e], p[c * 32 + 2 * e + 1]), f2_add(dp, lds_pair(ndlt + c * 32 + 2 * e)));
+          float d0, d1;
+          f2_unpack(dsv, d0, d1);
+          dk[e] = tc::pack_bf16(d0, d1);
+        }
+      } else {
+#pragma unroll
+        for (int e = 0; e < 16; ++e) dk[e] = 0u;
+      }
+      tc::tmem_st16(a.tDP + a.lane_off + a.half * 64 + c * 16, dk);
+      if (KEYTAIL && !a.key_live) {
+#pragma unroll
+        for (int e = 0; e < 16; ++e) dk[e] = 0u;
+      }
+#pragma unroll
+      for (int m = 0; m < 4; ++m)
+        sts128(ds_row ^ (uint32_t)((c * 4 + m) << 4), dk[4 * m], dk[4 * m + 1], dk[4 * m + 2], dk[4 * m + 3]);
+    }
+    tc::tmem_st_wait();
+  } else {
+#pragma unroll
+    for (int cc = 0; cc < 8; ++cc) sts128(ds_row ^ (uint32_t)(cc << 4), 0u, 0u, 0u, 0u);
+  }
+  tc::fence_proxy_async_smem();
+  tc::tc_fence_before();
+  tc::mbar_arrive(&s.ds_full);
+  if (a.half == 0 && a.row < 32) BWD_TRACE(1, i, 4);
+}
+
+template <int GMODE, bool KEYTAIL>
 __device__ __forceinline__ void bwd_softmax_loop(BwdSmem& s, const SoftmaxArgs& a, int T0) {
-  const int row = a.row, N = a.N;
-  const int wq = row & ~31;
   uint32_t cwn[16];
   auto load_codes = [&](int i) {
-    const uint4* src = reinterpret_cast<const uint4*>(a.code + (size_t)a.b * a.code_bs + (size_t)min(i * BM + row, N - 1) * a.code_ld + a.colbase);
+    const uint4* src = reinterpret_cast<const uint4*>(a.code + i * BM + a.half * 64);
 #pragma unroll
     for (int v = 0; v < 4; ++v) {
-      uint4 t = make_uint4(0u, 0u, 0u, 0u);
-      if (!TAIL || a.colbase + v * 16 < N) t = __ldg(src + v);
+      const uint4 t = __ldg(src + v);
       cwn[v * 4 + 0] = t.x; cwn[v * 4 + 1] = t.y; cwn[v * 4 + 2] = t.z; cwn[v * 4 + 3] = t.w;
     }
   };
@@ -184,52 +185,9 @@
       for (int v = 0; v < 16; ++v) cw[v] = cwn[v];
       if (i + 1 < a.ntiles) load_codes(i + 1);
     }
-    const int q0 = i * BM;
     const int T = T0 + i;
-    const int pds_par = (T > 0) ? ((T - 1) & 1) : -1;
-    const int qi = q0 + row;
-    const bool rows_live = q0 + wq < N;
-    float lse2 = INFINITY, dlt = 0.f;
-    if (rows_live) {
-      tc::mbar_wait(&s.stat_full[T & 1], (T >> 1) & 1);
-      lse2 = s.stat[T & 1][0][row];
-      dlt = s.stat[T & 1][1][row];
-    }
-    if (a.half == 0 && row < 32) BWD_TRACE(1, i, 0);
-    tc::mbar_wait(&s.sdp_full, T & 1);
-    tc::tc_fence_after();
-    if (a.half == 0 && row < 32) BWD_TRACE(1, i, 1);
-    if (!rows_live) {
-      tc::tc_fence_before();
-      tc::mbar_arrive(&s.sdp_free);
-      if (pds_par >= 0) {
-        tc::mbar_wait(&s.pds_free, (uint32_t)pds_par);
-        tc::mbar_wait(&s.dq_full, (uint32_t)pds_par);
-        tc::tc_fence_after();
-      }
-#pragma unroll
-      for (int cc = 0; cc < 8; ++cc) {
-        sts128(a.p_row ^ (uint32_t)(cc << 4), 0u, 0u, 0u, 0u);
-        sts128(a.ds_row ^ (uint32_t)(cc << 4), 0u, 0u, 0u, 0u);
-      }
-      {
-        uint32_t z[16];
-#pragma unroll
-        for (int e = 0; e < 16; ++e) z[e] = 0u;
-        tc::tmem_st16(a.tDS + a.lane_off + a.half * 32, z);
-        tc::tmem_st16(a.tDS + a.lane_off + a.half * 32 + 16, z);
-        tc::tmem_st_wait();
-      }
-    } else {
-      const float* grow = (GMODE == 1 || GMODE == 2) ? a.g_mean + (size_t)a.b * a.g_bs + (size_t)min(qi, N - 1) * a.g_ld + a.colbase : nullptr;
-      float* rd_row0 = (a.g_row0 != nullptr && qi == 0) ? a.g_row0 + ((size_t)a.b * a.H + a.h) * N + a.colbase : nullptr;
-      const float gw = (GMODE == 3) ? ((qi == 0) ? a.w_cls2 : a.w_aff2) : a.invH;
-      bwd_softmax_tile<GMODE, TAIL>(s, a.tS, a.tDP, a.tDS, a.lane_off, a.half, row, a.colbase, N, grow, cw, gw, a.scale_log2, lse2, dlt, rd_row0,
-                                    a.p_row, a.ds_row, pds_par);
-    }
-    tc::fence_proxy_async_smem();
-    tc::mbar_arrive(&s.pds_full);
-    if (a.half == 0 && row < 32) BWD_TRACE(1, i, 4);
+    if (a.warp_live) tc::mbar_wait(&s.stat_full[T & 1], (T >> 1) & 1);
+    bwd_softmax_tile<GMODE, KEYTAIL>(s, a, i, T, cw);
   }
 }
 
@@ -256,6 +214,8 @@
     return false;
   }
 };
+
+__device__ __forceinline__ uint32_t pT_col(int ks) { return (uint32_t)((ks >> 2) * 64 + (ks & 3) * 8); }
 
 __global__ void __launch_bounds__(BWD_THREADS, 1)
 attn_bwd_kernel(const __grid_constant__ CUtensorMap tmap_qkv, const __grid_constant__ CUtensorMap tmap_do,
@@ -286,13 +246,18 @@
       tc::mbar_init(&s.qdo_full[i], 1);
       tc::mbar_init(&s.qdo_empty[i], 1);
     }
-    for (int i = 0; i < 2; ++i) tc::mbar_init(&s.stat_full[i], 64);
-    tc::mbar_init(&s.sdp_full, 1);
-    tc::mbar_init(&s.sdp_free, 256);
-    tc::mbar_init(&s.pds_full, 256);
-    tc::mbar_init(&s.pds_free, 1);
-    tc::mbar_init(&s.dq_full, 1);
-    tc::mbar_init(&s.dq_free, 128);
+    tc::mbar_init(&s.s_full, 1);
+    tc::mbar_init(&s.dp_full, 1);
+    tc::mbar_init(&s.p_full, 256);
+    tc::mbar_init(&s.ds_full, 256);
+    tc::mbar_init(&s.p_done, 1);
+    tc::mbar_init(&s.dk_done, 1);
+    for (int i = 0; i < 2; ++i) {
+      tc::mbar_init(&s.stat_full[i], 64);
+      tc::mbar_init(&s.ds_free[i], 1);
+      tc::mbar_init(&s.dq_full[i], 1);
+      tc::mbar_init(&s.dq_free[i], 128);
+    }
     tc::fence_barrier_init();
   }
   if (warp == 2) tc::tmem_alloc<512>(&s.tmem_base);
@@ -301,7 +266,7 @@
   tc::tc_fence_after();
   if (warp == 0) BWD_TRACE(3, 0, 0);
   const uint32_t tmem = s.tmem_base;
-  const uint32_t tS = tmem, tDP = tmem + 128, tDV = tmem + 256, tDK = tmem + 320, tDQ = tmem + 384, tDS = tmem + 448;
+  const uint32_t tS = tmem, tDP = tmem + 128, tDV = tmem + 256, tDK = tmem + 320, tDQ = tmem + 384;
 
   if (warp < 4) {
     tc::reg_dealloc<REG_CTRL>();
@@ -332,20 +297,28 @@
       const uint64_t kd_k = tc::smem_desc_sw128(tc::smem_u32(s.k), 16, 1024);
       const uint64_t vd_k = tc::smem_desc_sw128(tc::smem_u32(s.v), 16, 1024);
       const uint64_t kd_mn = tc::smem_desc_sw128(tc::smem_u32(s.k), 1024, 1024);
-      const uint64_t pd_mn = tc::smem_desc_sw128(tc::smem_u32(s.p[0]), TILE_BYTES, 1024);
-      const uint64_t dsd_mn = tc::smem_desc_sw128(tc::smem_u32(s.ds[0]), TILE_BYTES, 1024);
-      auto issue_scores = [&](int T) {
+      auto issue_s = [&](int T) {
         const int st = T % NST;
         tc::mbar_wait(&s.qdo_full[st], (T / NST) & 1);
+        if (T > 0) tc::mbar_wait(&s.p_done, (T - 1) & 1);
         tc::tc_fence_after();
-        BWD_TRACE(0, T, 0);
-        const uint64_t qd = tc::smem_desc_sw128(tc::smem_u32(s.q[st]), 16, 1024), dod = tc::smem_desc_sw128(tc::smem_u32(s.d_o[st]), 16, 1024);
+        const uint64_t qd = tc::smem_desc_sw128(tc::smem_u32(s.q[st]), 16, 1024);
         if (tc::elect_one()) {
 #pragma unroll
-          for (int ks = 0; ks < HD / 16; ++ks) tc::mma_ss_off(tS, qd, ks * 2, kd_k, ks * 2, IDESC_S, ks > 0);
-#pragma unroll
-          for (int ks = 0; ks < HD / 16; ++ks) tc::mma_ss_off(tDP, dod, ks * 2, vd_k, ks * 2, IDESC_S, ks > 0);
-          tc::tc_commit(&s.sdp_full);
+          for (int ks = 0; ks < HD / 16; ++ks) tc::mma_ss_off(tS, kd_k, ks * 2, qd, ks * 2, IDESC_S, ks > 0);
+          tc::tc_commit(&s.s_full);
+        }
+        __syncwarp();
+      };
+      auto issue_dp = [&](int T) {
+        const int st = T % NST;
+        if (T > 0) tc::mbar_wait(&s.dk_done, (T - 1) & 1);
+        tc::tc_fence_after();
+        const uint64_t dod = tc::smem_desc_sw128(tc::smem_u32(s.d_o[st]), 16, 1024);
+        if (tc::elect_one()) {
+#pragma unroll
+          for (int ks = 0; ks < HD / 16; ++ks) tc::mma_ss_off(tDP, vd_k, ks * 2, dod, ks * 2, IDESC_S, ks > 0);
+          tc::tc_commit(&s.dp_full);
         }
         __syncwarp();
       };
@@ -353,39 +326,45 @@
       bool tail;
       for (int k = 0; items.at(cta, G, k, kvt, hb, tail); ++k) {
         tc::mbar_wait(&s.kv_full, k & 1);
-        if (T > 0) tc::mbar_wait(&s.sdp_free, (T - 1) & 1);
-        issue_scores(T);
+        issue_s(T);
+        issue_dp(T);
         for (int i = 0; i < ntiles; ++i, ++T) {
           const int st = T % NST;
-          if (i + 1 < ntiles) {
-            tc::mbar_wait(&s.sdp_free, T & 1);
-            issue_scores(T + 1);
-          }
           const uint64_t qd_mn = tc::smem_desc_sw128(tc::smem_u32(s.q[st]), 1024, 1024), dod_mn = tc::smem_desc_sw128(tc::smem_u32(s.d_o[st]), 1024, 1024);
-          BWD_TRACE(0, T, 1);
-          tc::mbar_wait(&s.pds_full, T & 1);
-          BWD_TRACE(0, T, 2);
-          if (T >= 1) tc::mbar_wait(&s.dq_free, (T - 1) & 1);
+          const uint64_t dsd_mn = tc::smem_desc_sw128(tc::smem_u32(s.ds[T & 1][0]), TILE_BYTES, 1024);
+          const uint32_t acc = (i > 0) ? 1u : 0u;
+          tc::mbar_wait(&s.p_full, T & 1);
+          BWD_TRACE(0, T, 0);
           if (i == 0 && k > 0) tc::mbar_wait(&s.dkv_free, (k - 1) & 1);
           tc::tc_fence_after();
-          const uint32_t acc = (i > 0) ? 1u : 0u;
           if (tc::elect_one()) {
 #pragma unroll
             for (int ks = 0; ks < BM / 16; ++ks)
-              tc::mma_ss_off(tDK, dsd_mn, ks * 128, qd_mn, ks * 128, IDESC_DQ, acc | (ks > 0));
+              tc::mma_ts_off(tDV, tS + pT_col(ks), dod_mn, ks * 128, IDESC_PV, acc | (ks > 0));
+            tc::tc_commit(&s.p_done);
+          }
+          __syncwarp();
+          if (i + 1 < ntiles) issue_s(T + 1);
+          tc::mbar_wait(&s.ds_full, T & 1);
+          BWD_TRACE(0, T, 1);
+          if (T >= 2) tc::mbar_wait(&s.dq_free[T & 1], ((T - 2) >> 1) & 1);
+          tc::tc_fence_after();
+          if (tc::elect_one()) {
 #pragma unroll
             for (int ks = 0; ks < BM / 16; ++ks)
-              tc::mma_ss_off(tDV, pd_mn, ks * 128, dod_mn, ks * 128, IDESC_DQ, acc | (ks > 0));
-            tc::tc_commit(&s.pds_free);
+              tc::mma_ts_off(tDK, tDP + pT_col(ks), qd_mn, ks * 128, IDESC_PV, acc | (ks > 0));
+            tc::tc_commit(&s.dk_done);
             tc::tc_commit(&s.qdo_empty[st]);
 #pragma unroll
             for (int ks = 0; ks < BN / 16; ++ks)
-              tc::mma_ts_off(tDQ, tDS + ks * 8, kd_mn, ks * 128, IDESC_PV, ks > 0);
-            tc::tc_commit(&s.dq_full);
+              tc::mma_ss_off(tDQ + (T & 1) * 64, dsd_mn, ks * 128, kd_mn, ks * 128, IDESC_DQ, ks > 0);
+            tc::tc_commit(&s.dq_full[T & 1]);
+            tc::tc_commit(&s.ds_free[T & 1]);
             if (i + 1 == ntiles) tc::tc_commit(&s.kv_empty);
           }
           __syncwarp();
-          BWD_TRACE(0, T, 3);
+          if (i + 1 < ntiles) issue_dp(T + 1);
+          BWD_TRACE(0, T, 2);
         }
       }
     } else {
@@ -403,7 +382,7 @@
             v[q] = (qi < N) ? __ldg(src + qi) : (which == 0 ? INFINITY : 0.f);
           }
 #pragma unroll
-          for (int q = 0; q < 4; ++q) s.stat[T & 1][which][q * 32 + lane] = (which == 0) ? v[q] * kLog2e : v[q];
+          for (int q = 0; q < 4; ++q) s.stat[T & 1][which][q * 32 + lane] = (which == 0) ? -v[q] * kLog2e : -v[q];
           tc::mbar_arrive(&s.stat_full[T & 1]);
         }
       }
@@ -415,21 +394,29 @@
     const int half = we >> 2;
     const uint32_t lane_off = (uint32_t)((warp & 3) * 32) << 16;
     const float invH = 1.f / (float)H;
-    const bool g_vec = (g_mean != nullptr) && ((g_ld & 3) == 0) && ((g_bs & 3) == 0) && ((reinterpret_cast<uintptr_t>(g_mean) & 15) == 0);
     float w_cls2 = 0.f, w_aff2 = 0.f;
     if (has_code) {
       const float sc = gc.scale ? __ldg(gc.scale) : 1.f;
       w_cls2 = 2.f * invH * sc * gc.w_cls;
       w_aff2 = 2.f * invH * sc * gc.w_aff;
     }
-    const uint32_t swz = (uint32_t)(row & 7) << 4;
-    const uint32_t p_row = (tc::smem_u32(s.p[half]) + row * 128) ^ swz, ds_row = (tc::smem_u32(s.ds[half]) + row * 128) ^ swz;
+    const uint32_t ds_row = (tc::smem_u32(s.ds[0][half]) + row * 128) ^ ((uint32_t)(row & 7) << 4);
     int T = 0, k = 0, kvt, hb;
     bool tail;
     auto run = [&](auto body, bool want_tail) {
       while (items.at(cta, G, k, kvt, hb, tail) && tail == want_tail) {
-        const SoftmaxArgs sa{tS, tDP, tDS, lane_off, half, row, kvt * BN + half * 64, N, H, ntiles, hb / H, hb % H, g_mean, g_bs, g_ld, g_row0,
-                             gc.ptr, gc.bs, gc.ld, w_cls2, w_aff2, invH, scale_log2, p_row, ds_row, swz};
+        const int b = hb / H, key = kvt * BN + row, keyc = min(key, N - 1);
+        SoftmaxArgs sa;
+        sa.tS = tS; sa.tDP = tDP; sa.lane_off = lane_off;
+        sa.half = half; sa.row = row; sa.key = key; sa.N = N; sa.H = H; sa.ntiles = ntiles; sa.b = b; sa.h = hb % H;
+        sa.warp_live = kvt * BN + (warp & 3) * 32 < N;
+        sa.key_live = key < N;
+        sa.g_col = g_mean ? g_mean + (size_t)b * g_bs + keyc : nullptr;
+        sa.g_ld = g_ld;
+        sa.g_row0 = g_row0;
+        sa.code = has_code ? gc.ptr + (size_t)b * gc.bs + (size_t)keyc * gc.ld : nullptr;
+        sa.w_cls2 = w_cls2; sa.w_aff2 = w_aff2; sa.invH = invH; sa.scale_log2 = scale_log2;
+        sa.ds_row = ds_row;
         body(sa, T);
         T += ntiles;
         ++k;
@@ -438,11 +425,8 @@
     if (has_code) {
       run([&](const SoftmaxArgs& sa, int T0) { bwd_softmax_loop<3, false>(s, sa, T0); }, false);
       run([&](const SoftmaxArgs& sa, int T0) { bwd_softmax_loop<3, true>(s, sa, T0); }, true);
-    } else if (g_mean != nullptr && g_vec) {
-      run([&](const SoftmaxArgs& sa, int T0) { bwd_softmax_loop<2, false>(s, sa, T0); }, false);
-      run([&](const SoftmaxArgs& sa, int T0) { bwd_softmax_loop<1, true>(s, sa, T0); }, true);
     } else if (g_mean != nullptr) {
-      run([&](const SoftmaxArgs& sa, int T0) { bwd_softmax_loop<1, true>(s, sa, T0); }, false);
+      run([&](const SoftmaxArgs& sa, int T0) { bwd_softmax_loop<1, false>(s, sa, T0); }, false);
       run([&](const SoftmaxArgs& sa, int T0) { bwd_softmax_loop<1, true>(s, sa, T0); }, true);
     } else {
       run([&](const SoftmaxArgs& sa, int T0) { bwd_softmax_loop<0, false>(s, sa, T0); }, false);
@@ -483,18 +467,19 @@
     bool tail;
     for (int k = 0; items.at(cta, G, k, kvt, hb, tail); ++k) {
       for (int i = 0; i < ntiles; ++i, ++T) {
+        const uint32_t tq = tDQ + (T & 1) * 64;
         if (warp == 12) BWD_TRACE(2, T, 0);
-        tc::mbar_wait(&s.dq_full, T & 1);
+        tc::mbar_wait(&s.dq_full[T & 1], (T >> 1) & 1);
         tc::tc_fence_after();
         if (warp == 12) BWD_TRACE(2, T, 1);
-        tc::tmem_ld32(tDQ + lane_off, r);
+        tc::tmem_ld32(tq + lane_off, r);
         tc::tmem_ld_wait();
         drain_box(0, 0, 0, i, hb);
         drain_box(16, 1, 16, i, hb);
-        tc::tmem_ld32(tDQ + lane_off + 32, r);
+        tc::tmem_ld32(tq + lane_off + 32, r);
         tc::tmem_ld_wait();
         tc::tc_fence_before();
-        tc::mbar_arrive(&s.dq_free);
+        tc::mbar_arrive(&s.dq_free[T & 1]);
         if (warp == 12) BWD_TRACE(2, T, 2);
         drain_box(0, 0, 32, i, hb);
         drain_box(16, 1, 48, i, hb);
diff --git a/acr_wsss_b200/csrc/attn_tc.cu b/acr_wsss_b200/csrc/attn_tc.cu
--- a/acr_wsss_b200/csrc/attn_tc.cu
+++ b/acr_wsss_b200/csrc/attn_tc.cu
@@ -558,6 +558,28 @@
   }
 }
 
+constexpr int CT = 64;
+__global__ void __launch_bounds__(256)
+bwd_code_transpose_kernel(const unsigned char* __restrict__ code, long long bs, long long ld, unsigned char* __restrict__ out, int ldt, int N) {
+  __shared__ uint32_t tile[CT][CT / 4 + 1];
+  const int q0 = blockIdx.x * CT, k0 = blockIdx.y * CT, b = blockIdx.z;
+  const int t = threadIdx.x, r = t >> 2, part = t & 3;
+  uint4 v = make_uint4(0u, 0u, 0u, 0u);
+  if (q0 + r < N) v = __ldg(reinterpret_cast<const uint4*>(code + (size_t)b * bs + (size_t)(q0 + r) * ld + k0) + part);
+  tile[r][part * 4 + 0] = v.x; tile[r][part * 4 + 1] = v.y; tile[r][part * 4 + 2] = v.z; tile[r][part * 4 + 3] = v.w;
+  __syncthreads();
+  if (k0 + r >= N) return;
+  uint32_t w[4];
+#pragma unroll
+  for (int j = 0; j < 4; ++j) {
+    uint32_t x = 0;
+#pragma unroll
+    for (int m = 0; m < 4; ++m) x |= ((tile[part * 16 + j * 4 + m][r >> 2] >> ((r & 3) * 8)) & 0xffu) << (m * 8);
+    w[j] = x;
+  }
+  *reinterpret_cast<uint4*>(out + ((size_t)b * N + k0 + r) * ldt + q0 + part * 16) = make_uint4(w[0], w[1], w[2], w[3]);
+}
+
 __global__ void __launch_bounds__(256)
 bwd_dq_convert_kernel(const long long* __restrict__ dq_acc, const int* __restrict__ dq_bad, __nv_bfloat16* __restrict__ d_qkv, int B, int N,
                       int H, float scale) {
@@ -591,7 +613,7 @@
   if (B <= 0 || N <= 0 || H <= 0 || D <= 0) return 0;
   const size_t rows = (size_t)B * H * N, kt = (N + BN - 1) / BN;
   return acr::align_up(rows * sizeof(float), 256) + acr::align_up(rows * D * sizeof(long long), 256) + acr::align_up(kt * rows * sizeof(float), 256) +
-         acr::align_up(rows * sizeof(int), 256);
+         acr::align_up(rows * sizeof(int), 256) + acr::align_up((size_t)B * N * (kt * BN), 256);
 }
 
 extern "C" int acr_attn_bwd_bf16(const void* qkv, const void* out, const float* lse, const void* d_out,
@@ -622,6 +644,7 @@
   long long* dq_acc = (long long*)((char*)workspace + acr::align_up(rows * sizeof(float), 256));
   float* delta_part = (float*)((char*)dq_acc + acr::align_up(rows * D * sizeof(long long), 256));
   int* dq_bad = (int*)((char*)delta_part + acr::align_up((size_t)kt * rows * sizeof(float), 256));
+  unsigned char* code_t = (unsigned char*)dq_bad + acr::align_up(rows * sizeof(int), 256);
   CUtensorMap tmap_qkv, tmap_do, tmap_dq;
   if (int e = make_tmap(&tmap_qkv, qkv, B, N, 3 * H, D)) return e;
   if (int e = make_tmap(&tmap_do, d_out, B, N, H, D)) return e;
@@ -651,7 +674,18 @@
   bwd_delta_kernel<<<(unsigned)((rows + 31) / 32), 256, 0, st>>>((const __nv_bfloat16*)out, (const __nv_bfloat16*)d_out, delta_part,
                                                                with_g ? kt : 0, delta, reinterpret_cast<float4*>(dq_acc), dq_bad, (long long)rows, N, H);
   if (int e = acr::check_launch("bwd_delta_kernel")) return e;
-  if (int e = launch_attn_bwd(tmap_qkv, tmap_do, tmap_dq, lse, delta, g_mean, g_batch_stride, g_row_stride, gc, (__nv_bfloat16*)d_qkv, g_row0, dq_bad, B, N, H, scale, st))
+  GCode gc_t = gc;
+  if (g_code) {
+    const int ldt = kt * BN;
+    dim3 grid(ldt / CT, (N + CT - 1) / CT, B);
+    acr::KernelTimer kt_("bwd_code_transpose_kernel", st);
+    bwd_code_transpose_kernel<<<grid, 256, 0, st>>>(g_code, code_batch_stride, code_row_stride, code_t, ldt, N);
+    if (int e = acr::check_launch("bwd_code_transpose_kernel")) return e;
+    gc_t.ptr = code_t;
+    gc_t.bs = (long long)N * ldt;
+    gc_t.ld = ldt;
+  }
+  if (int e = launch_attn_bwd(tmap_qkv, tmap_do, tmap_dq, lse, delta, g_mean, g_batch_stride, g_row_stride, gc_t, (__nv_bfloat16*)d_qkv, g_row0, dq_bad, B, N, H, scale, st))
     return e;
   const long long nconv = (long long)rows * (HD / 8);
   bwd_dq_convert_kernel<<<(unsigned)((nconv + 255) / 256), 256, 0, st>>>(dq_acc, dq_bad, (__nv_bfloat16*)d_qkv, B, N, H, scale);
```

After: 577.0, median of 6. 1.5% lower.
